# oxfordcontrol/COSMO.jl

Hardware: AMD Instinct MI355X
Metric: ADMM iterations/sec (fp64) at fixed (n,m,nnz,cone) (higher is better)
Workload: dtype f64

## Files before the change

cosmo.jl_amd/_ffi.py:

```python
from __future__ import annotations

import ctypes as C
import os

import numpy as np

_HERE = os.path.dirname(os.path.abspath(__file__))
LIB_PATH = os.path.join(_HERE, "libcosmo_hip.so")
LIB_PATH_F32 = os.path.join(_HERE, "libcosmo_hip_f32.so")

OK = 0
ERR_NAMES = {1: "INVALID", 2: "HIP", 5: "EIG", 6: "UNSUPPORTED", 7: "COMM"}

ZERO, NONNEG, BOX, SOC, PSD_SQUARE, PSD_TRIANGLE = 0, 1, 2, 3, 4, 5
EXP, DUAL_EXP, POW, DUAL_POW = 6, 7, 8, 9
PSD_TRIANGLE_COMPLEX = 10
CUSTOM = 11
KKT_CG, KKT_MINRES_REDUCED, KKT_MINRES, KKT_CG_SR, KKT_CG_JACOBI = 0, 1, 2, 3, 4
KKT_DIRECT = 5
STATUS_NAMES = {0: "Undetermined", 1: "Solved", 2: "Max_iter_reached", 3: "Unsolved", 4: "Primal_infeasible",
                5: "Dual_infeasible", 6: "Time_limit_reached"}
MAT_A, MAT_AT, MAT_P, MAT_OP = 0, 1, 2, 3
MAX_RHO_UPDATES = 64
NUM_KERNEL_CLASSES = 16


from ._abi_structs import ABI_VERSION, AccelParams, Params, ResultStruct

ACCEL_EMPTY, ACCEL_ANDERSON = 0, 1
PSD_PROJECTION_SIGN, PSD_PROJECTION_EIGEN = 0, 1
ACCEL_ANDERSON_TYPE1_RESTARTED, ACCEL_ANDERSON_TYPE1_ROLLING, ACCEL_ANDERSON_TYPE2NE_RESTARTED, ACCEL_ANDERSON_TYPE2NE_ROLLING = 2, 3, 4, 5


class CosmoHipError(RuntimeError):
    def __init__(self, code, msg):
        super().__init__("libcosmo_hip error %d (%s): %s" % (code, ERR_NAMES.get(code, "?"), msg))
        self.code = code


_libs = {}

_PD = C.POINTER(C.c_double)
_PF = C.POINTER(C.c_float)


class _RealPtr:
    """Placeholder in SIGNATURES for `cosmo_hip_real*` (include/cosmo_hip.h): resolved to double* or float* when a library is loaded."""


_PR = _RealPtr
_PI64 = C.POINTER(C.c_int64)
_PI32 = C.POINTER(C.c_int32)

PROJECT_FN = C.CFUNCTYPE(None, C.POINTER(C.c_double), C.c_int64, C.c_void_p)
CONE_TEST_FN = C.CFUNCTYPE(C.c_int32, C.POINTER(C.c_double), C.c_int64, C.c_double, C.c_void_p)
PROJECT_FN_F32 = C.CFUNCTYPE(None, C.POINTER(C.c_float), C.c_int64, C.c_void_p)
CONE_TEST_FN_F32 = C.CFUNCTYPE(C.c_int32, C.POINTER(C.c_float), C.c_int64, C.c_double, C.c_void_p)

SIGNATURES = {
    "cosmo_hip_version": (C.c_int32, []),
    "cosmo_hip_default_params": (None, [C.POINTER(Params)]),
    "cosmo_hip_create": (C.c_int32, [C.POINTER(C.c_void_p), C.c_int32]),
    "cosmo_hip_destroy": (C.c_int32, [C.c_void_p]),
    "cosmo_hip_last_error": (C.c_char_p, [C.c_void_p]),
    "cosmo_hip_set_problem": (C.c_int32, [C.c_void_p, C.c_int64, C.c_int64, _PI64, _PI64, _PR, _PI64, _PI64, _PR, _PR, _PR]),
    "cosmo_hip_set_cones": (C.c_int32, [C.c_void_p, C.c_int64, _PI32, _PI64, _PR, _PR]),
    "cosmo_hip_set_cones_ex": (C.c_int32, [C.c_void_p, C.c_int64, _PI32, _PI64, _PR, _PR, _PR]),
    "cosmo_hip_set_custom_cone": (C.c_int32, [C.c_void_p, C.c_int64, PROJECT_FN, CONE_TEST_FN, CONE_TEST_FN, C.c_void_p]),
    "cosmo_hip_set_params": (C.c_int32, [C.c_void_p, C.POINTER(Params), _PR]),
    "cosmo_hip_update_rho": (C.c_int32, [C.c_void_p, _PR]),
    "cosmo_hip_set_scaling": (C.c_int32, [C.c_void_p, _PR, _PR, C.c_double]),
    "cosmo_hip_set_scaling_full": (C.c_int32, [C.c_void_p, _PR, _PR, _PR, _PR, C.c_double, C.c_double]),
    "cosmo_hip_default_accel_params": (None, [C.POINTER(AccelParams)]),
    "cosmo_hip_set_accelerator": (C.c_int32, [C.c_void_p, C.POINTER(AccelParams)]),
    "cosmo_hip_get_accel_stats": (C.c_int32, [C.c_void_p, _PI64]),
    "cosmo_hip_get_accel_restarts": (C.c_int32, [C.c_void_p, _PI64]),
    "cosmo_hip_scale_ruiz": (C.c_int32, [C.c_void_p, C.c_int64, C.c_double, C.c_double, _PR, _PR, _PD]),
    "cosmo_hip_update_qb": (C.c_int32, [C.c_void_p, _PR, _PR]),
    "cosmo_hip_get_rho_classes": (C.c_int32, [C.c_void_p, _PI32]),
    "cosmo_hip_get_rho_vec": (C.c_int32, [C.c_void_p, _PR]),
    "cosmo_hip_kkt_solve": (C.c_int32, [C.c_void_p, _PR, _PR, _PI64]),
    "cosmo_hip_project": (C.c_int32, [C.c_void_p, _PR, _PI64, _PI32]),
    "cosmo_hip_spmv": (C.c_int32, [C.c_void_p, C.c_int32, _PR, _PR]),
    "cosmo_hip_set_iterates": (C.c_int32, [C.c_void_p, _PR, _PR, _PR]),
    "cosmo_hip_admm_init": (C.c_int32, [C.c_void_p]),
    "cosmo_hip_admm_iterate": (C.c_int32, [C.c_void_p, C.c_int64]),
    "cosmo_hip_admm_iterate_checked": (C.c_int32, [C.c_void_p, C.c_int64, _PI32]),
    "cosmo_hip_residuals": (C.c_int32, [C.c_void_p, _PD]),
    "cosmo_hip_optimize": (C.c_int32, [C.c_void_p, C.POINTER(ResultStruct)]),
    "cosmo_hip_get_iterates": (C.c_int32, [C.c_void_p, _PR, _PR, _PR, _PR]),
    "cosmo_hip_cg_persist_stats": (C.c_int32, [C.c_void_p, _PI64]),
    "cosmo_hip_fold_stats": (C.c_int32, [C.c_void_p, _PI64]),
    "cosmo_hip_kkt_recurrence": (C.c_char_p, [C.c_void_p]),
    "cosmo_hip_ldl_analyze": (C.c_int32, [C.c_int64, C.c_int64, _PI64, _PI64, _PI64, _PI64, _PI64, _PI64]),
    "cosmo_hip_set_kkt_perm": (C.c_int32, [C.c_void_p, C.c_int64, _PI64]),
    "cosmo_hip_direct_info": (C.c_int32, [C.c_void_p, _PI64]),
    "cosmo_hip_polar_dataflow_stats": (C.c_int32, [C.c_void_p, _PD]),
    "cosmo_hip_polar_dataflow_reset_timing": (C.c_int32, [C.c_void_p]),
    "cosmo_hip_get_kkt_solution": (C.c_int32, [C.c_void_p, _PR]),
    "cosmo_hip_get_stats": (C.c_int32, [C.c_void_p, _PI64]),
    "cosmo_hip_set_setup_time": (C.c_int32, [C.c_void_p, C.c_double]),
    "cosmo_hip_get_rho_interval": (C.c_int32, [C.c_void_p, _PI64]),
    "cosmo_hip_time_spmv": (C.c_int32, [C.c_void_p, C.c_int32, C.c_int32, _PD, _PD]),
    "cosmo_hip_set_profiling": (C.c_int32, [C.c_void_p, C.c_int32]),
    "cosmo_hip_get_kernel_times": (C.c_int32, [C.c_void_p, _PD, _PI64]),
    "cosmo_hip_kernel_class_name": (C.c_char_p, [C.c_int32]),
    "cosmo_hip_psd_stats": (C.c_int32, [C.c_void_p, _PI64]),
    "cosmo_hip_set_psd_projection": (C.c_int32, [C.c_void_p, C.c_int32]),
    "cosmo_hip_polar_stats": (C.c_int32, [C.c_void_p, _PI64]),
    "cosmo_hip_polar_streamk_stats": (C.c_int32, [C.c_void_p, _PI64]),
    "cosmo_hip_polar_schedule": (C.c_int32, [C.c_int32, _PD, _PI32]),
    "cosmo_hip_time_psd_product": (C.c_int32, [C.c_void_p, C.c_int32, C.c_int32, _PD, _PD]),
    "cosmo_hip_comm_unique_id": (C.c_int32, [C.POINTER(C.c_uint8)]),
    "cosmo_hip_comm_init": (C.c_int32, [C.c_void_p, C.c_int32, C.c_int32, C.POINTER(C.c_uint8)]),
    "cosmo_hip_comm_destroy": (C.c_int32, [C.c_void_p]),
    "cosmo_hip_set_cone_shard": (C.c_int32, [C.c_void_p, _PI64]),
    "cosmo_hip_polar_depth_stats": (C.c_int32, [C.c_void_p, _PI64]),
    "cosmo_hip_time_krylov": (C.c_int32, [C.c_void_p, C.c_int32, C.POINTER(C.c_double), C.POINTER(C.c_double), C.POINTER(C.c_int32)]),
    "cosmo_hip_comm_selftest": (C.c_int32, [C.c_void_p]),
    "cosmo_hip_comm_allreduce_check": (C.c_int32, [C.c_void_p, C.c_int64, _PI64]),
    "cosmo_hip_comm_init_hostshm": (C.c_int32, [C.c_void_p, C.c_int32, C.c_int32, C.c_char_p]),
    "cosmo_hip_comm_stats": (C.c_int32, [C.c_void_p, _PI64]),
    "cosmo_hip_set_cone_ownership": (C.c_int32, [C.c_void_p, C.c_int64, C.c_int64]),
    "cosmo_hip_set_row_shard": (C.c_int32, [C.c_void_p, _PI64]),
    "cosmo_hip_row_shard_info": (C.c_int32, [C.c_void_p, _PI64]),
    "cosmo_hip_comm_stats_ex": (C.c_int32, [C.c_void_p, _PI64]),
    "cosmo_hip_batch_create": (C.c_int32, [C.POINTER(C.c_void_p), C.c_int32, C.c_int64, C.c_int64, C.c_int64]),
    "cosmo_hip_batch_destroy": (C.c_int32, [C.c_void_p]),
    "cosmo_hip_batch_last_error": (C.c_char_p, [C.c_void_p]),
    "cosmo_hip_batch_set_problem": (C.c_int32, [C.c_void_p, C.c_int64, _PI64, _PI64, _PR, _PI64, _PI64, _PR, _PR, _PR]),
    "cosmo_hip_batch_set_cones": (C.c_int32, [C.c_void_p, C.c_int64, _PI32, _PI64, _PR, _PR]),
    "cosmo_hip_batch_set_cones_ex": (C.c_int32, [C.c_void_p, C.c_int64, _PI32, _PI64, _PR, _PR, _PR]),
    "cosmo_hip_batch_set_scaling": (C.c_int32, [C.c_void_p, C.c_int64, _PR, _PR, C.c_double]),
    "cosmo_hip_batch_set_params": (C.c_int32, [C.c_void_p, C.POINTER(Params)]),
    "cosmo_hip_batch_set_accelerator": (C.c_int32, [C.c_void_p, C.POINTER(AccelParams)]),
    "cosmo_hip_batch_get_accel_stats": (C.c_int32, [C.c_void_p, _PI64]),
    "cosmo_hip_batch_get_rho_classes": (C.c_int32, [C.c_void_p, C.c_int64, _PI32]),
    "cosmo_hip_batch_set_iterates": (C.c_int32, [C.c_void_p, _PR, _PR, _PR]),
    "cosmo_hip_batch_optimize": (C.c_int32, [C.c_void_p, C.POINTER(ResultStruct)]),
    "cosmo_hip_batch_iterate": (C.c_int32, [C.c_void_p, C.c_int64, C.c_int32]),
    "cosmo_hip_batch_get_iterates": (C.c_int32, [C.c_void_p, C.c_int64, _PR, _PR, _PR, _PR]),
    "cosmo_hip_batch_get_counters": (C.c_int32, [C.c_void_p, _PI64]),
    "cosmo_hip_batch_kernel_info": (C.c_int32, [C.c_void_p, _PI64]),
    "cosmo_hip_batch_set_direct": (C.c_int32, [C.c_void_p, C.c_int32, _PI64]),
    "cosmo_hip_batch_direct_info": (C.c_int32, [C.c_void_p, _PI64]),
    "cosmo_hip_batch_direct_counts": (C.c_int32, [C.c_void_p, _PI64]),
    "cosmo_hip_batch_set_scaling_full": (C.c_int32, [C.c_void_p, C.c_int64, _PR, _PR, _PR, _PR, C.c_double, C.c_double]),
    "cosmo_hip_batch_stage_qb": (C.c_int32, [C.c_void_p, C.c_int64, _PR, _PR]),
    "cosmo_hip_batch_apply_updates": (C.c_int32, [C.c_void_p]),
    "cosmo_hip_batch_update_qb": (C.c_int32, [C.c_void_p, C.c_int64, _PI64, _PR, _PR]),
    "cosmo_hip_batch_warm_restart": (C.c_int32, [C.c_void_p]),
    "cosmo_hip_batch_get_qb": (C.c_int32, [C.c_void_p, C.c_int64, _PR, _PR]),
    "cosmo_hip_batch_group_create": (C.c_int32, [C.POINTER(C.c_void_p), C.c_int32, C.c_int64]),
    "cosmo_hip_batch_group_destroy": (C.c_int32, [C.c_void_p]),
    "cosmo_hip_batch_group_last_error": (C.c_char_p, [C.c_void_p]),
    "cosmo_hip_batch_group_set_problem": (C.c_int32, [C.c_void_p, C.c_int64, C.c_int64, C.c_int64, _PI64, _PI64, _PR, _PI64, _PI64, _PR, _PR, _PR]),
    "cosmo_hip_batch_group_set_cones": (C.c_int32, [C.c_void_p, C.c_int64, C.c_int64, _PI32, _PI64, _PR, _PR, _PR]),
    "cosmo_hip_batch_group_set_scaling": (C.c_int32, [C.c_void_p, C.c_int64, _PR, _PR, C.c_double]),
    "cosmo_hip_batch_group_set_scaling_full": (C.c_int32, [C.c_void_p, C.c_int64, _PR, _PR, _PR, _PR, C.c_double, C.c_double]),
    "cosmo_hip_batch_group_set_accelerator": (C.c_int32, [C.c_void_p, C.POINTER(AccelParams)]),
    "cosmo_hip_batch_group_set_direct": (C.c_int32, [C.c_void_p, C.c_int32]),
    "cosmo_hip_batch_group_set_params": (C.c_int32, [C.c_void_p, C.POINTER(Params)]),
    "cosmo_hip_batch_group_class_info": (C.c_int32, [C.c_void_p, _PI64, _PI64, _PI64]),
    "cosmo_hip_batch_group_run_info": (C.c_int32, [C.c_void_p, _PI64]),
    "cosmo_hip_batch_group_get_rho_interval": (C.c_int32, [C.c_void_p, C.c_int64, _PI64]),
# ... 153 lines not shown
            if fn is None:
                return test_t(0)
            return test_t(lambda ptr, dim, tol, _user: 1 if fn(_view(ptr, dim), float(tol)) else 0)

        f32 = self.dtype == np.float32
        proj_t, test_t = (PROJECT_FN_F32, CONE_TEST_FN_F32) if f32 else (PROJECT_FN, CONE_TEST_FN)
        thunks = (proj_t(_proj), _mk(in_dual), _mk(in_pol_recc))
        self._callbacks[int(cone)] = thunks
        self._chk(self.lib.cosmo_hip_set_custom_cone(self._h, int(cone), thunks[0], thunks[1], thunks[2], None))

    def default_params(self):
        return default_params(self.dtype)

    def set_params(self, params, rho_vec=None):
        rv = self._f(rho_vec, self.m, "rho_vec")
        self._chk(self.lib.cosmo_hip_set_params(self._h, C.byref(params), _dp(rv)))

    def update_rho(self, rho_vec):
        rv = self._f(rho_vec, self.m, "rho_vec")
        self._chk(self.lib.cosmo_hip_update_rho(self._h, _dp(rv)))

    def set_accelerator(self, kind=ACCEL_ANDERSON, mem=15, min_mem=3, safeguard=True, safeguard_tol=2.0, start_iter=2, start_accuracy=None):
        ap = AccelParams()
        self.lib.cosmo_hip_default_accel_params(C.byref(ap))
        ap.kind, ap.mem, ap.min_mem, ap.safeguard = int(kind), int(mem), int(min_mem), 1 if safeguard else 0
        ap.safeguard_tol, ap.start_iter = float(safeguard_tol), int(start_iter)
        if start_accuracy is not None:
            ap.start_accuracy = float(start_accuracy)
        self._chk(self.lib.cosmo_hip_set_accelerator(self._h, C.byref(ap)))

    def accel_restarts(self):
        out = np.zeros(2, dtype=np.int64)
        self._chk(self.lib.cosmo_hip_get_accel_restarts(self._h, out.ctypes.data_as(_PI64)))
        return int(out[0]), int(out[1])

    def set_psd_projection(self, mode):
        self._chk(self.lib.cosmo_hip_set_psd_projection(self._h, int(mode)))

    def accel_stats(self):
        out = np.zeros(6, dtype=np.int64)
        self._chk(self.lib.cosmo_hip_get_accel_stats(self._h, out.ctypes.data_as(_PI64)))
        return dict(accelerated=int(out[0]), accepted=int(out[1]), declined=int(out[2]), restarts=int(out[3]), active=bool(out[4]),
                    safeguarding_iter=int(out[5]))

    def scale_ruiz(self, iterations, min_scaling=1e-4, max_scaling=1e4):
        D = np.empty(self.n, dtype=self.dtype); E = np.empty(self.m, dtype=self.dtype); c = C.c_double(1.0)
        self._chk(self.lib.cosmo_hip_scale_ruiz(self._h, int(iterations), float(min_scaling), float(max_scaling), _dp(D), _dp(E), C.byref(c)))
        return D, E, float(c.value)

    def set_scaling(self, Dinv, Einv, cinv):
        self._chk(self.lib.cosmo_hip_set_scaling(self._h, _dp(self._f(Dinv, self.n)), _dp(self._f(Einv, self.m)), float(cinv)))

    def set_scaling_full(self, D, Dinv, E, Einv, c, cinv):
        self._chk(self.lib.cosmo_hip_set_scaling_full(self._h, _dp(self._f(D, self.n)), _dp(self._f(Dinv, self.n)), _dp(self._f(E, self.m)),
                                                      _dp(self._f(Einv, self.m)), float(c), float(cinv)))

    def update_qb(self, q=None, b=None):
        self._chk(self.lib.cosmo_hip_update_qb(self._h, _dp(self._f(q, self.n)), _dp(self._f(b, self.m))))

    def get_rho_classes(self):
        out = np.empty(self.m, dtype=np.int32)
        self._chk(self.lib.cosmo_hip_get_rho_classes(self._h, out.ctypes.data_as(_PI32)))
        return out

    def get_rho_vec(self):
        out = np.empty(self.m, dtype=self.dtype)
        self._chk(self.lib.cosmo_hip_get_rho_vec(self._h, _dp(out)))
        return out

    def kkt_solve(self, rhs):
        rhs = self._f(rhs, self.n + self.m, "rhs")
        lhs = np.empty(self.n + self.m, dtype=self.dtype)
        it = C.c_int64(0)
        self._chk(self.lib.cosmo_hip_kkt_solve(self._h, _dp(lhs), _dp(rhs), C.byref(it)))
        return lhs, it.value

    def project(self, s):
        s = np.array(s, dtype=self.dtype).copy()
        ranks = np.empty(max(self.ncones, 1), dtype=np.int64)
        br = np.empty(max(self.ncones, 1), dtype=np.int32)
        self._chk(self.lib.cosmo_hip_project(self._h, _dp(s), ranks.ctypes.data_as(_PI64), br.ctypes.data_as(_PI32)))
        return s, ranks[:self.ncones], br[:self.ncones]

    def spmv(self, which, x):
        nin = {MAT_A: self.n, MAT_AT: self.m, MAT_P: self.n}[which]
        nout = {MAT_A: self.m, MAT_AT: self.n, MAT_P: self.n}[which]
        x = self._f(x, nin, "x")
        y = np.empty(nout, dtype=self.dtype)
        self._chk(self.lib.cosmo_hip_spmv(self._h, which, _dp(y), _dp(x)))
        return y

    def set_iterates(self, x0=None, s0=None, mu0=None):
        self._chk(self.lib.cosmo_hip_set_iterates(self._h, _dp(self._f(x0, self.n)), _dp(self._f(s0, self.m)), _dp(self._f(mu0, self.m))))

    def admm_init(self):
        self._chk(self.lib.cosmo_hip_admm_init(self._h))

    def admm_iterate(self, n_iters):
        self._chk(self.lib.cosmo_hip_admm_iterate(self._h, int(n_iters)))

    def admm_iterate_checked(self, n_iters):
        st = C.c_int32(0)
        self._chk(self.lib.cosmo_hip_admm_iterate_checked(self._h, int(n_iters), C.byref(st)))
        return st.value

    def set_setup_time(self, seconds):
        self._chk(self.lib.cosmo_hip_set_setup_time(self._h, float(seconds)))

    def rho_interval(self):
        out = np.zeros(2, dtype=np.int64)
        self._chk(self.lib.cosmo_hip_get_rho_interval(self._h, out.ctypes.data_as(_PI64)))
        return int(out[0]), int(out[1])

    def residuals(self):
        out = np.empty(5)
        self._chk(self.lib.cosmo_hip_residuals(self._h, _dp(out)))
        return out

    def optimize(self):
        r = ResultStruct()
        self._chk(self.lib.cosmo_hip_optimize(self._h, C.byref(r)))
        return r

    def get_iterates(self):
        N = self.n + self.m
        w = np.empty(N, dtype=self.dtype); wp = np.empty(N, dtype=self.dtype); s = np.empty(self.m, dtype=self.dtype); mu = np.empty(self.m, dtype=self.dtype)
        self._chk(self.lib.cosmo_hip_get_iterates(self._h, _dp(w), _dp(wp), _dp(s), _dp(mu)))
        return w, wp, s, mu

    def get_kkt_solution(self):
        sol = np.empty(self.n + self.m, dtype=self.dtype)
        self._chk(self.lib.cosmo_hip_get_kkt_solution(self._h, _dp(sol)))
        return sol

    def get_stats(self):
        out = np.zeros(8, dtype=np.int64)
        self._chk(self.lib.cosmo_hip_get_stats(self._h, out.ctypes.data_as(_PI64)))
        keys = ["admm_iters", "kkt_solves", "kkt_iters_total", "kkt_budget_stalls", "spmv_A", "spmv_AT", "spmv_P", "rho_updates"]
        return dict(zip(keys, out.tolist()))

    def cg_persist_stats(self):
        out = np.zeros(8, dtype=np.int64)
        self._chk(self.lib.cosmo_hip_cg_persist_stats(self._h, out.ctypes.data_as(_PI64)))
        return dict(zip(["enabled", "workgroups", "launches", "fallbacks", "tickets", "arrivals", "abort", "lds_per_quarter"], out.tolist()))

    def set_kkt_perm(self, perm):
        if perm is None:
            self._chk(self.lib.cosmo_hip_set_kkt_perm(self._h, 0, None))
            return
        p = np.ascontiguousarray(perm, dtype=np.int64)
        self._chk(self.lib.cosmo_hip_set_kkt_perm(self._h, int(p.size), p.ctypes.data_as(_PI64)))

    def direct_info(self):
        out = np.zeros(8, dtype=np.int64)
        self._chk(self.lib.cosmo_hip_direct_info(self._h, out.ctypes.data_as(_PI64)))
        keys = ["nnz_L", "nnz_stored", "supernodes", "height", "max_width", "factorizations", "positive_pivots", "last_factor_ns"]
        return dict(zip(keys, out.tolist()))

    def kkt_recurrence(self):
        return self.lib.cosmo_hip_kkt_recurrence(self._h).decode()

    def fold_stats(self):
        out = np.zeros(6, dtype=np.int64)
        self._chk(self.lib.cosmo_hip_fold_stats(self._h, out.ctypes.data_as(_PI64)))
        return dict(zip(["enabled", "nnz", "terms", "tiles", "factored_rows", "stored_entries"], out.tolist()))

# ... 389 lines not shown
```

cosmo.jl_amd/csrc/api.hip:

```cpp
#include <stdarg.h>
#include <stdio.h>
#include <string.h>
#include <math.h>
#include <algorithm>
#include <chrono>
#include "internal.h"
#include "device_utils.h"

int32_t cosmo_fail(cosmo_hip_handle* h, int32_t code, const char* fmt, ...) {
  char buf[1024];
  va_list ap;
  va_start(ap, fmt);
  vsnprintf(buf, sizeof buf, fmt, ap);
  va_end(ap);
  if (h) h->err = buf;
  return code;
}

template <class T>
static int32_t dalloc(cosmo_hip_handle* h, T** p, size_t count) {
  if (*p) { (void)hipFree(*p); *p = nullptr; }
  if (count == 0) count = 1;
  HIPCHK(h, hipMalloc((void**)p, count * sizeof(T)));
  HIPCHK(h, hipMemsetAsync(*p, 0, count * sizeof(T), h->stream));
// ... 577 lines not shown
}

extern "C" int32_t cosmo_hip_update_qb(cosmo_hip_handle* h, const real* q, const real* b) {
  ENTER(h);
  if (!h->have_problem) return cosmo_fail(h, COSMO_HIP_ERR_INVALID, "set_problem first");
  if (b && h->row_shard) return cosmo_fail(h, COSMO_HIP_ERR_UNSUPPORTED, "update_qb(b): not available on a row-sharded handle");
  if (q) CHK(h2d(h, h->q, q, (size_t)h->n));
  if (b) {
    CHK(h2d(h, h->b, b, (size_t)h->m));
    if (h->have_cones) {
      std::vector<real> bhost(b, b + h->m);
      CHK(classify_rows(h, bhost));
    }
  }
  return COSMO_HIP_OK;
}

extern "C" int32_t cosmo_hip_get_rho_classes(cosmo_hip_handle* h, int32_t* cls) {
  ENTER(h);
  if (h->row_shard) return cosmo_fail(h, COSMO_HIP_ERR_UNSUPPORTED, "get_rho_classes: not available on a row-sharded handle");
  if (!h->have_cones || !cls) return cosmo_fail(h, COSMO_HIP_ERR_INVALID, "get_rho_classes: not set up");
  return d2h(h, cls, h->rho_cls, (size_t)h->m);
}
extern "C" int32_t cosmo_hip_get_rho_vec(cosmo_hip_handle* h, real* rho_vec) {
  ENTER(h);
  if (h->row_shard) return cosmo_fail(h, COSMO_HIP_ERR_UNSUPPORTED, "get_rho_vec: not available on a row-sharded handle");
  if (!h->have_params || !rho_vec) return cosmo_fail(h, COSMO_HIP_ERR_INVALID, "get_rho_vec: not set up");
  return d2h(h, rho_vec, h->rho, (size_t)h->m);
}

int32_t sync_ctl(cosmo_hip_handle* h) {
  HIPCHK(h, hipMemcpyAsync(h->ctl_host, h->ctl, sizeof(Ctl), hipMemcpyDeviceToHost, h->stream));
  HIPCHK(h, hipStreamSynchronize(h->stream));
  CHK(prof_collect(h));
  if (h->ctl_host->error) return cosmo_fail(h, h->ctl_host->error, "device raised error %d", h->ctl_host->error);
  return COSMO_HIP_OK;
}

extern "C" int32_t cosmo_hip_spmv(cosmo_hip_handle* h, int32_t which, real* y, const real* x) {
  ENTER(h);
  if (h->row_shard) return cosmo_fail(h, COSMO_HIP_ERR_UNSUPPORTED, "spmv: not available on a row-sharded handle");
  if (!h->have_problem || !x || !y) return cosmo_fail(h, COSMO_HIP_ERR_INVALID, "spmv: not set up");
  const CsrDev* M = which == COSMO_HIP_MAT_A ? &h->A : which == COSMO_HIP_MAT_AT ? &h->AT : which == COSMO_HIP_MAT_P ? &h->P : nullptr;
  if (!M) return cosmo_fail(h, COSMO_HIP_ERR_INVALID, "spmv: bad matrix id");
  real* dx = h->io;
  real* dy = h->io + M->ncols;
  if ((long long)M->ncols + M->nrows > 2 * (h->n + h->m)) return cosmo_fail(h, COSMO_HIP_ERR_INVALID, "spmv: staging too small");
  CHK(h2d(h, dx, x, (size_t)M->ncols));
  CHK(launch_spmv_plain(h, *M, dx, dy));
  CHK(d2h(h, y, dy, (size_t)M->nrows));
  h->spmv_calls[which] += 1;
  return COSMO_HIP_OK;
}

extern "C" int32_t cosmo_hip_project(cosmo_hip_handle* h, real* s, int64_t* psd_rank_out, int32_t* soc_branch_out) {
  ENTER(h);
  if (h->row_shard) return cosmo_fail(h, COSMO_HIP_ERR_UNSUPPORTED, "project: not available on a row-sharded handle");
  if (!h->have_cones || (!s && h->m > 0)) return cosmo_fail(h, COSMO_HIP_ERR_INVALID, "project: not set up");
  CHK(h2d(h, h->io, s, (size_t)h->m));
  CHK(launch_project_simple_inplace(h, h->io));
  CHK(launch_soc(h, h->io, 0));
  CHK(cone3_enqueue_project(h, h->io, 0));
  CHK(psd_enqueue_project(h, h->io, false));
  CHK(custom_enqueue_project(h, h->io, 0));
  CHK(comm_enqueue_exchange(h, h->io));
  CHK(d2h(h, s, h->io, (size_t)h->m));
  const size_t nc = h->cones.type.size();
  if (soc_branch_out) {
    for (size_t k = 0; k < nc; ++k) soc_branch_out[k] = -1;
    if (h->nsoc) {
      std::vector<int> br((size_t)h->nsoc);
      CHK(d2h(h, br.data(), h->soc_branch, (size_t)h->nsoc));
      for (int i = 0; i < h->nsoc; ++i) soc_branch_out[h->soc_cone_index[i]] = br[i];
    }
    CHK(cone3_get_branches(h, soc_branch_out));
  }
  if (psd_rank_out) {
    for (size_t k = 0; k < nc; ++k) psd_rank_out[k] = -1;
    CHK(psd_get_ranks(h, psd_rank_out));
    for (size_t k = 0; k < nc; ++k)
      if ((h->cones.type[k] == COSMO_HIP_PSD_SQUARE || h->cones.type[k] == COSMO_HIP_PSD_TRIANGLE) && h->cones.dim[k] == 1)
        psd_rank_out[k] = s[h->cones.off[k]] > R(0.0) ? 1 : 0;
  }
  return COSMO_HIP_OK;
}

static void adapt_budget(cosmo_hip_handle* h) {
  const int kmax = h->ctl_host->cg_k_max;
  int nb = kmax + 2;
  if (nb < 3) nb = 3;
  if (nb > 4096) nb = 4096;
  h->budget = nb;
}

__global__ void k_ctl_reset_kmax(Ctl* ctl) { ctl->cg_k_max = 0; }
__global__ void k_ctl_set_status(Ctl* ctl, int st) { ctl->status = st; ctl->halt = 1; }
static bool inf_due(const cosmo_hip_handle* h, long long it);

static int32_t maybe_infeas_check(cosmo_hip_handle* h, long long it) {
  if (h->ctl_host->status != 0 || !inf_due(h, it)) return COSMO_HIP_OK;
  int32_t st = 0;
  CHK(infeas_check(h, &st));
  if (st != 0) {
    hipLaunchKernelGGL(k_ctl_set_status, dim3(1), dim3(1), 0, h->stream, h->ctl, st);
    CHK(sync_ctl(h));
  }
  return COSMO_HIP_OK;
}

extern "C" int32_t cosmo_hip_kkt_solve(cosmo_hip_handle* h, real* lhs, const real* rhs, int64_t* kkt_iters_out) {
  ENTER(h);
  if (h->row_shard) return cosmo_fail(h, COSMO_HIP_ERR_UNSUPPORTED, "kkt_solve: not available on a row-sharded handle");
  if (!h->have_params || !lhs || !rhs) return cosmo_fail(h, COSMO_HIP_ERR_INVALID, "kkt_solve: not set up");
  CHK(h2d(h, h->ls_x, rhs, (size_t)h->n));
  CHK(h2d(h, h->ls_s, rhs + h->n, (size_t)h->m));
  CHK(kkt_solve_now(h));
  h->host_solves += 1;
  CHK(sync_ctl(h));
  if (kkt_iters_out) *kkt_iters_out = h->ctl_host->cg_k;
  CHK(d2h(h, lhs, h->x_tl, (size_t)h->n));
  CHK(d2h(h, lhs + h->n, h->nu, (size_t)h->m));
  return COSMO_HIP_OK;
}

extern "C" int32_t cosmo_hip_set_iterates(cosmo_hip_handle* h, const real* x0, const real* s0, const real* mu0) {
  ENTER(h);
  if (!h->have_params) return cosmo_fail(h, COSMO_HIP_ERR_INVALID, "set_iterates: set_params first");
  const long long n = h->n, m = h->m;
  const real *dx = nullptr, *ds = nullptr, *dm = nullptr;
  if (h->row_shard) { if (s0) s0 += h->row_lo; if (mu0) mu0 += h->row_lo; }
  if (x0) { CHK(h2d(h, h->ls_x, x0, (size_t)n)); dx = h->ls_x; }
  if (s0) { CHK(h2d(h, h->ls_s, s0, (size_t)m)); ds = h->ls_s; }
  if (mu0) { CHK(h2d(h, h->tmp_m, mu0, (size_t)m)); dm = h->tmp_m; }
  CHK(launch_set_w(h, dx, ds, dm));
  HIPCHK(h, hipMemcpyAsync(h->w_prev, h->w, sizeof(real) * (size_t)(n + m), hipMemcpyDeviceToDevice, h->stream));
  CHK(d2h(h, h->ctl_host, h->ctl, 1));
  Ctl* c = h->ctl_host;
  c->halt = 0; c->status = 0; c->stalled = 0; c->error = 0; c->cg_done = 0; c->cg_k = 0; c->cg_k_max = 0; c->rho_changed = 0;
  c->iter = 0;
  c->r_prim = INFINITY; c->r_dual = INFINITY; c->max_norm_prim = 0; c->max_norm_dual = 0; c->cost = INFINITY;
  CHK(h2d(h, h->ctl, h->ctl_host, 1));
  h->host_iter = 0;
  h->have_iterates = true;
  h->fb_from = h->fb_recorded;
  return COSMO_HIP_OK;
}

static const int FB_LAG = 2;
static void feedback_reset(cosmo_hip_handle* h) { h->fb_from = h->fb_recorded; }
int32_t solve_budget(cosmo_hip_handle* h, int* budget_out) {
  const int R = cosmo_hip_handle::FB_RING;
  bool& used = h->fb_used[(h->host_solves + 1) % R];
  used = false;
  if (h->fb_mode == 1 && !h->fb_k) {
    if (const char* e = getenv("COSMO_HIP_BUDGET_FEEDBACK")) { if (atoi(e) == 0) h->fb_mode = 0; }
    if (h->fb_mode == 1 && hipHostMalloc((void**)&h->fb_k, sizeof(int) * cosmo_hip_handle::FB_RING) != hipSuccess) { (void)hipGetLastError(); h->fb_k = nullptr; h->fb_mode = 0; }
  }
  *budget_out = h->budget;
  if (h->fb_mode != 1 || h->profiling || h->exact_launches) return COSMO_HIP_OK;
  const long long j = h->fb_recorded - FB_LAG;
  const int wide = h->budget + h->budget / 16;
  if (j < h->fb_from || j < 0) { *budget_out = wide > 4096 ? 4096 : wide; return COSMO_HIP_OK; }
  HIPCHK(h, hipEventSynchronize(h->fb_ev[j % R]));
  int kmax = h->fb_k[j % R], kmin = kmax, nv = 1;
  for (long long i = j - 1; i >= h->fb_from && i > j - 4; --i) { const int v = h->fb_k[i % R]; kmax = std::max(kmax, v); kmin = std::min(kmin, v); nv += 1; }
  int b = (nv >= 3) ? kmax + (kmax - kmin) / 2 + kmax / 40 + 3 : kmax + (kmax * 15 + 99) / 100 + 6;
// ... 506 lines not shown
```

cosmo.jl_amd/csrc/internal.h:

```cpp
#pragma once
#include <hip/hip_runtime.h>
#include <stdint.h>
#include <string>
#include <vector>
#include "../../include/cosmo_hip.h"

typedef cosmo_hip_real real;
#ifdef COSMO_HIP_REAL_FLOAT
typedef float2 real2;
#define make_real2 make_float2
#define REAL_EPS 1.1920928955078125e-07f
#define REAL_MAX 3.402823466e+38f
#define REAL_IS_FLOAT 1
#else
typedef double2 real2;
#define make_real2 make_double2
#define REAL_EPS 2.220446049250313e-16
#define REAL_MAX 1.7976931348623157e308
#define REAL_IS_FLOAT 0
#endif
#define R(x) ((real)(x))

#define COSMO_BS 256
#define COSMO_NNZ_PER_BLOCK 2048
// ... 257 lines not shown
int32_t launch_set_w(cosmo_hip_handle* h, const real* x0, const real* s0, const real* mu0);
int32_t launch_recover_mu(cosmo_hip_handle* h);
int32_t launch_rho_from_classes(cosmo_hip_handle* h, real rho0);
int32_t launch_spmv_plain(cosmo_hip_handle* h, const CsrDev& M, const real* x, real* y);
int32_t launch_spmv_A_rho(cosmo_hip_handle* h, int guard, int mode, const real* v, real* out);
int32_t launch_reduced_rhs(cosmo_hip_handle* h, int guard, real* out_rhs);
int32_t launch_cg_upd(cosmo_hip_handle* h, int guard, int k, int n_uc);
int32_t launch_cg_dir_check(cosmo_hip_handle* h, int guard, int kk, int n_rr);
int32_t enqueue_cg_rhs(cosmo_hip_handle* h, int guard);
int32_t enqueue_cg_start(cosmo_hip_handle* h, int guard, real tol_k);
int32_t enqueue_cg_iterations(cosmo_hip_handle* h, int guard, int k_begin, int count);
int32_t enqueue_rhs(cosmo_hip_handle* h, int guard);
int32_t enqueue_y2_only(cosmo_hip_handle* h);
int32_t enqueue_tail(cosmo_hip_handle* h, int loop_mode);
int32_t enqueue_count_solve(cosmo_hip_handle* h);
int32_t enqueue_clear_stall(cosmo_hip_handle* h);
int32_t enqueue_check(cosmo_hip_handle* h, int guard, int mode);
int32_t time_op_apply(cosmo_hip_handle* h, int reps, double* avg_seconds);

int32_t fold_build(cosmo_hip_handle* h, const HostCsr& Am, const std::vector<int>& prp, const std::vector<int>& pcol,
                   const std::vector<real>& pval, int factor_min);
int32_t fold_refresh(cosmo_hip_handle* h);
void fold_free(cosmo_hip_handle* h);
int32_t fold_enqueue_start(cosmo_hip_handle* h, int guard, real tol_k);
int32_t fold_enqueue_iterations(cosmo_hip_handle* h, int guard, int k_begin, int count);

int32_t minres_alloc(cosmo_hip_handle* h);
int32_t minres_enqueue_solve(cosmo_hip_handle* h, int guard, bool from_loop);
int32_t minres_resume(cosmo_hip_handle* h, int extra);
int32_t launch_mr_tail_full(cosmo_hip_handle* h, int loop_mode, const real* xsol);

int32_t ldl_setup(cosmo_hip_handle* h, const std::vector<int64_t>& perm_req);
void ldl_free(cosmo_hip_handle* h);
int32_t ldl_enqueue_refactor(cosmo_hip_handle* h, int cond);
int32_t ldl_refactor_now(cosmo_hip_handle* h, bool inertia);
int32_t ldl_enqueue_solve(cosmo_hip_handle* h, int guard, bool from_loop);
int32_t ldl_info(cosmo_hip_handle* h, int64_t* out);

int32_t sr_alloc(cosmo_hip_handle* h);
void sr_free(cosmo_hip_handle* h);
int32_t sr_enqueue_start(cosmo_hip_handle* h, int guard);
int32_t sr_enqueue_iterations(cosmo_hip_handle* h, int guard, int k_begin, int count);

bool batch_multi_supported(const cosmo_hip_batch* b);
bool batch_multi_needs_ext(const cosmo_hip_batch* b);
int32_t batch_multi_optimize(cosmo_hip_batch** bs, int count, bool ext, cosmo_hip_result* results);

int32_t pcg_setup(cosmo_hip_handle* h, bool* accepted);
void pcg_free(cosmo_hip_handle* h);
int32_t pcg_enqueue_solve(cosmo_hip_handle* h, int guard);

void aa_free(cosmo_hip_handle* h);
bool aa_get_params(const cosmo_hip_handle* h, cosmo_hip_accel_params* out);
bool aa_enabled(const cosmo_hip_handle* h);
bool aa_safeguarded(const cosmo_hip_handle* h);
bool aa_active(const cosmo_hip_handle* h);
int32_t aa_restart(cosmo_hip_handle* h);
void aa_note_rho_restart(cosmo_hip_handle* h);
int32_t aa_begin_solve(cosmo_hip_handle* h);
int32_t aa_enqueue_pre(cosmo_hip_handle* h, long long it, bool* attempted);
int32_t aa_fetch_flags(cosmo_hip_handle* h, int* success, int* declined);
int32_t aa_enqueue_guard(cosmo_hip_handle* h);
int32_t aa_enqueue_reset(cosmo_hip_handle* h);
void aa_count(cosmo_hip_handle* h, int accelerated, int declined);
void aa_check_accuracy_activation(cosmo_hip_handle* h, real r_prim, real r_dual, real max_norm_prim, real max_norm_dual);

int32_t cone3_plan_create(cosmo_hip_handle* h);
void cone3_free(cosmo_hip_handle* h);
int32_t cone3_enqueue_project(cosmo_hip_handle* h, real* s, int guard);
int32_t cone3_enqueue_in_dual_neg(cosmo_hip_handle* h, const real* v, real tol, int* flag);
int32_t cone3_get_branches(cosmo_hip_handle* h, int32_t* out_per_cone);

int32_t custom_plan_create(cosmo_hip_handle* h);
void custom_free(cosmo_hip_handle* h);
int32_t custom_enqueue_project(cosmo_hip_handle* h, real* s, int guard);
int32_t custom_test(cosmo_hip_handle* h, const real* v_dev, int which, real tol, bool* ok);

int32_t polar_plan_create(cosmo_hip_handle* h);
void polar_plan_destroy(cosmo_hip_handle* h);
bool polar_enabled(const cosmo_hip_handle* h);
int32_t polar_enqueue_project(cosmo_hip_handle* h, real* s, int guard);
int32_t polar_enqueue_project_batch(cosmo_hip_handle* h, real* s, int guard);
int32_t polar_adapt(cosmo_hip_handle* h);
bool polar_has_batch(const cosmo_hip_handle* h);
bool polar_has_large(const cosmo_hip_handle* h);

int32_t polar_complex_is_pd(cosmo_hip_handle* h, const real* vec, real sign, real tol, std::vector<int>& ok);

int32_t psd_plan_create(cosmo_hip_handle* h);
void psd_plan_destroy(cosmo_hip_handle* h);
int32_t psd_enqueue_project(cosmo_hip_handle* h, real* s, bool guard);
int32_t psd_get_ranks(cosmo_hip_handle* h, int64_t* rank_per_cone);
int32_t psd_extreme_eigs(cosmo_hip_handle* h, const real* vec, real sign, real tol, std::vector<real>& lam_min);
static inline bool cone_owned(const cosmo_hip_handle* h, long long k) { return h->cone_hi < 0 || (k >= h->cone_lo && k < h->cone_hi); }
int32_t infeas_enqueue_capture(cosmo_hip_handle* h);
int32_t infeas_check(cosmo_hip_handle* h, int32_t* status);
int32_t comm_enqueue_exchange(cosmo_hip_handle* h, real* s);
int32_t comm_allgather_rows(cosmo_hip_handle* h, real* full);
int32_t comm_allreduce_sum(cosmo_hip_handle* h, real* buf, size_t count);
int32_t comm_allreduce_host(cosmo_hip_handle* h, double* vals, int count, int op );
int comm_nranks(const cosmo_hip_handle* h);
int comm_rank(const cosmo_hip_handle* h);
int32_t comm_allreduce_flag(cosmo_hip_handle* h, int* flag);
int32_t comm_set_partition(cosmo_hip_handle* h, const int64_t* first_cone, const char* who);
void comm_my_range(const cosmo_hip_handle* h, long long* cone_lo, long long* cone_hi, long long* row_lo, long long* row_hi);
int32_t rs_enqueue_cg_rhs(cosmo_hip_handle* h, int guard);
int32_t rs_get_iterates(cosmo_hip_handle* h, real* w, real* w_prev, real* s, real* mu);
void rs_free(cosmo_hip_handle* h);
extern "C" int32_t cosmo_hip_comm_destroy(cosmo_hip_handle* h);
```

cosmo.jl_amd/csrc/psd.hip:

```cpp
#include "device_utils.h"
#include <algorithm>
#include <math.h>
#include <stdlib.h>

#include "psd_internal.h"
#include "psd16.h"
#include "psdwg.h"

__global__ __launch_bounds__(COSMO_BS) void k_psd_tiny(const Ctl* __restrict__ ctl, int guard, int ncones,
                                                       const int* __restrict__ list, const PsdConeDev* __restrict__ cones,
                                                       real* __restrict__ s, int* __restrict__ rank, int* __restrict__ flags,
                                                       int mode, real sign, real* __restrict__ eigmin) {
  if (guard && ctl->halt) return;
  __shared__ __attribute__((aligned(16))) unsigned char wsb[COSMO_BS / 64][(PSD16_WS_BYTES + 15) / 16 * 16];
  const int lane = threadIdx.x & 63, wv = threadIdx.x >> 6;
  const int widx = blockIdx.x * (COSMO_BS / 64) + wv;
  if (widx >= ncones) return;
  const PsdConeDev cn = cones[list[widx]];
  const Psd16Ws ws = psd16_ws_at(wsb[wv]);
  int nonconv = 0;
  real lm = 0.0;
  const int rk = psd16_wave(s + cn.off, cn.d, cn.kind, ws, lane, mode, sign, &lm, &nonconv);
  if (nonconv && lane == 0) atomicOr(&flags[1], 1);
  if (mode == 1) { if (lane == 0) eigmin[list[widx]] = lm; return; }
// ... 313 lines not shown
      p->d_pj_groups.push_back(dptr);
    }
  }
  HIPCHK(h, hipMalloc((void**)&p->G, std::max<long long>(1, p->gsize) * sizeof(real)));
  HIPCHK(h, hipMalloc((void**)&p->colw, std::max(1, p->ncolw) * sizeof(real)));
  HIPCHK(h, hipMalloc((void**)&p->cshift, p->cones.size() * sizeof(real)));
  HIPCHK(h, hipMalloc((void**)&p->rank, p->cones.size() * sizeof(int)));
  HIPCHK(h, hipMalloc((void**)&p->flags, 4 * sizeof(int)));
  HIPCHK(h, hipMalloc((void**)&p->eigmin, p->cones.size() * sizeof(real)));
  HIPCHK(h, hipMemset(p->rank, 0, p->cones.size() * sizeof(int)));
  HIPCHK(h, hipMemset(p->flags, 0, 4 * sizeof(int)));
  return polar_plan_create(h);
}

static int32_t psd_large_sweeps(cosmo_hip_handle* h, int n, int nbmax) {
  PsdPlan* p = h->psd;
  int sweep = 0;
  for (; sweep < PSD_MAX_SWEEPS; ++sweep) {
    HIPCHK(h, hipMemsetAsync(p->flags, 0, sizeof(int), h->stream));
    for (int st = -1; st < nbmax - 1; ++st)
      hipLaunchKernelGGL(k_psd_step, dim3(nbmax / 2, n), dim3(PSD_STEP_WAVES * 64), 0, h->stream, p->d_large, p->d_cones, p->G,
                         p->cshift, st, p->flags, p->tol_factor);
    int fl = 0;
    HIPCHK(h, hipMemcpyAsync(&fl, p->flags, sizeof(int), hipMemcpyDeviceToHost, h->stream));
    HIPCHK(h, hipStreamSynchronize(h->stream));
    if (!fl) break;
  }
  p->last_large_sweeps = sweep + 1;
  if (sweep >= PSD_MAX_SWEEPS) return cosmo_fail(h, COSMO_HIP_ERR_EIG, "Jacobi eigensolver did not converge in %d sweeps", PSD_MAX_SWEEPS);
  return COSMO_HIP_OK;
}

bool psd_needs_sync(const cosmo_hip_handle* h) { return h->psd && !h->psd->large.empty() && !polar_has_large(h); }

int32_t psd_enqueue_project(cosmo_hip_handle* h, real* s, bool guard_b) {
  PsdPlan* p = h->psd;
  if (!p || p->cones.empty()) return COSMO_HIP_OK;
  const int guard = guard_b ? 1 : 0;
  prof_begin(h, KC_PSD);
  HIPCHK(h, hipMemsetAsync(p->rank, 0, p->cones.size() * sizeof(int), h->stream));
  if (!p->tiny.empty()) {
    const int n = (int)p->tiny.size();
    hipLaunchKernelGGL(k_psd_tiny, dim3((n + COSMO_BS / 64 - 1) / (COSMO_BS / 64)), dim3(COSMO_BS), 0, h->stream, h->ctl, guard, n,
                       p->d_tiny, p->d_cones, s, p->rank, p->flags, 0, 1.0, p->eigmin);
  }
  for (size_t gi = 0; gi < p->pj_groups.size(); ++gi) {
    const int n = (int)p->pj_groups[gi].size();
    const int* lst = p->d_pj_groups[gi];
    hipLaunchKernelGGL(k_psd_populate, dim3(8, n), dim3(COSMO_BS), 0, h->stream, h->ctl, guard, lst, p->d_cones, s, p->G, p->cshift, 1.0, 0);
    switch (p->pj_waves[gi]) {
      case 16: hipLaunchKernelGGL((k_psd_jacobi_wg<16>), dim3(n), dim3(1024), 0, h->stream, h->ctl, guard, lst, p->d_cones, p->G, p->cshift, p->flags, p->tol_factor, p->dbg); break;
      default: hipLaunchKernelGGL((k_psd_jacobi_wg<4>), dim3(n), dim3(256), 0, h->stream, h->ctl, guard, lst, p->d_cones, p->G, p->cshift, p->flags, p->tol_factor, p->dbg); break;
    }
    hipLaunchKernelGGL(k_psd_colscale, dim3(4, n), dim3(COSMO_BS), 0, h->stream, h->ctl, guard, lst, p->d_cones, p->G, p->cshift, p->colw, p->rank);
    int maxtiles = 1;
    for (int idx : p->pj_groups[gi]) { const int nt = p->cones[idx].ld / 16; maxtiles = std::max(maxtiles, nt * (nt + 1) / 2); }
    hipLaunchKernelGGL(k_psd_syrk, dim3((maxtiles + 3) / 4, n), dim3(COSMO_BS), 0, h->stream, h->ctl, guard, lst, p->d_cones, p->G, s);
  }
  if (polar_has_batch(h)) CHK(polar_enqueue_project_batch(h, s, guard));
  if (polar_has_large(h)) CHK(polar_enqueue_project(h, s, guard));
  if (!p->large.empty() && !(polar_has_large(h) && p->large_by_polar)) {
    if (guard) {
      CHK(sync_ctl(h));
      if (h->ctl_host->halt) { prof_end(h); return COSMO_HIP_OK; }
    }
    const int n = (int)p->large.size();
    int nbmax = 0;
    for (int idx : p->large) nbmax = std::max(nbmax, p->cones[idx].nb);
    hipLaunchKernelGGL(k_psd_populate, dim3(64, n), dim3(COSMO_BS), 0, h->stream, h->ctl, 0, p->d_large, p->d_cones, s, p->G, p->cshift, 1.0, 0);
    CHK(psd_large_sweeps(h, n, nbmax));
    hipLaunchKernelGGL(k_psd_colscale, dim3(128, n), dim3(COSMO_BS), 0, h->stream, h->ctl, 0, p->d_large, p->d_cones, p->G, p->cshift, p->colw, p->rank);
    int maxtiles = 1;
    for (int idx : p->large) { const int nt = p->cones[idx].ld / 16; maxtiles = std::max(maxtiles, nt * (nt + 1) / 2); }
    hipLaunchKernelGGL(k_psd_syrk, dim3(std::min(8192, (maxtiles + 3) / 4), n), dim3(COSMO_BS), 0, h->stream, h->ctl, 0, p->d_large, p->d_cones, p->G, s);
  }
  prof_end(h);
  HIPCHK(h, hipGetLastError());
  return COSMO_HIP_OK;
}

int32_t psd_get_ranks(cosmo_hip_handle* h, int64_t* rank_per_cone) {
  PsdPlan* p = h->psd;
  if (!p || p->cones.empty()) return COSMO_HIP_OK;
  std::vector<int> r(p->cones.size());
  int fl[4] = {0, 0, 0, 0};
  HIPCHK(h, hipMemcpyAsync(r.data(), p->rank, r.size() * sizeof(int), hipMemcpyDeviceToHost, h->stream));
  HIPCHK(h, hipMemcpyAsync(fl, p->flags, sizeof fl, hipMemcpyDeviceToHost, h->stream));
  HIPCHK(h, hipStreamSynchronize(h->stream));
  if (fl[1]) return cosmo_fail(h, COSMO_HIP_ERR_EIG, "Jacobi eigensolver did not converge");
  for (size_t i = 0; i < p->cones.size(); ++i) rank_per_cone[p->cones[i].cone_index] = r[i];
  return COSMO_HIP_OK;
}

extern "C" int32_t cosmo_hip_psd_stats(cosmo_hip_handle* h, int64_t out[4]) {
  if (!h || !out) return COSMO_HIP_ERR_INVALID;
  out[0] = out[1] = out[2] = out[3] = 0;
  PsdPlan* p = h->psd;
  if (!p || p->cones.empty()) return COSMO_HIP_OK;
  int fl[4] = {0, 0, 0, 0};
  HIPCHK(h, hipMemcpyAsync(fl, p->flags, sizeof fl, hipMemcpyDeviceToHost, h->stream));
  HIPCHK(h, hipStreamSynchronize(h->stream));
  out[0] = fl[2]; out[1] = p->last_large_sweeps; out[2] = fl[1]; out[3] = (int64_t)p->cones.size();
  return COSMO_HIP_OK;
}


int32_t psd_extreme_eigs(cosmo_hip_handle* h, const real* vec, real sign, real tol, std::vector<real>& lam_min) {
  PsdPlan* p = h->psd;
  lam_min.clear();
  if (!p || p->cones.empty()) return COSMO_HIP_OK;
  real* v = const_cast<real*>(vec);
  if (!p->tiny.empty()) {
    const int n = (int)p->tiny.size();
    hipLaunchKernelGGL(k_psd_tiny, dim3((n + COSMO_BS / 64 - 1) / (COSMO_BS / 64)), dim3(COSMO_BS), 0, h->stream, h->ctl, 0, n, p->d_tiny,
                       p->d_cones, v, p->rank, p->flags, 1, sign, p->eigmin);
  }
  for (size_t gi = 0; gi < p->wg_groups.size(); ++gi) {
    const int n = (int)p->wg_groups[gi].size();
    const int* lst = p->d_wg_groups[gi];
    hipLaunchKernelGGL(k_psd_populate, dim3(8, n), dim3(COSMO_BS), 0, h->stream, h->ctl, 0, lst, p->d_cones, vec, p->G, p->cshift, sign, 1);
    if (p->wg_waves[gi] == 16)
      hipLaunchKernelGGL((k_psd_jacobi_wg<16>), dim3(n), dim3(1024), 0, h->stream, h->ctl, 0, lst, p->d_cones, p->G, p->cshift, p->flags, p->tol_factor, 0);
    else
      hipLaunchKernelGGL((k_psd_jacobi_wg<4>), dim3(n), dim3(256), 0, h->stream, h->ctl, 0, lst, p->d_cones, p->G, p->cshift, p->flags, p->tol_factor, 0);
    hipLaunchKernelGGL(k_psd_eigmin, dim3(n), dim3(COSMO_BS), 0, h->stream, lst, p->d_cones, p->G, p->cshift, p->eigmin);
  }
  if (!p->large.empty()) {
    const int n = (int)p->large.size();
    int nbmax = 0;
    for (int idx : p->large) nbmax = std::max(nbmax, p->cones[idx].nb);
    hipLaunchKernelGGL(k_psd_populate, dim3(64, n), dim3(COSMO_BS), 0, h->stream, h->ctl, 0, p->d_large, p->d_cones, vec, p->G, p->cshift, sign, 1);
    CHK(psd_large_sweeps(h, n, nbmax));
    hipLaunchKernelGGL(k_psd_eigmin, dim3(n), dim3(COSMO_BS), 0, h->stream, p->d_large, p->d_cones, p->G, p->cshift, p->eigmin);
  }
  HIPCHK(h, hipGetLastError());
  lam_min.resize(p->cones.size());
  HIPCHK(h, hipMemcpyAsync(lam_min.data(), p->eigmin, sizeof(real) * lam_min.size(), hipMemcpyDeviceToHost, h->stream));
  HIPCHK(h, hipStreamSynchronize(h->stream));
  if (!p->cplx.empty()) {
    std::vector<int> ok;
    CHK(polar_complex_is_pd(h, vec, sign, tol, ok));
    for (size_t q = 0; q < p->cplx.size(); ++q) lam_min[p->cplx[q]] = ok[q] ? 0.0 : -INFINITY;
  }
  return COSMO_HIP_OK;
}
```

cosmo.jl_amd/csrc/psd_polar.hip:

```cpp
#include "psd_internal.h"
#include <math.h>
#include <stdlib.h>
#include <string.h>
#include <algorithm>
#include <mutex>

#define PK 16
#ifndef POLAR_PREFETCH_DEPTH
#define POLAR_PREFETCH_DEPTH 2
#endif
#define PLD 80

struct PolarCone {
  int idx;
  int off, d, kind;
  int ts;
  int sk;
  int skg, skc;
  int ld;
  long long woff;
};

struct BatchCone { long long woff; int off, d, kind, ld, idx, ts; };

struct SkSync { unsigned ticket; unsigned timeout; unsigned pad[14]; unsigned flag[1]; };
struct PolarDev {
  int gate;
  int rounds;
  int verified;
  int unverified;
  int projections;
  int pad[3];
  real err_last, err_max;
};

static const real kPolarLift[3] = {3.8438259784376458, -2.5414431444903771, 0.42553478492344637};
#define POLAR_NFIN 5
static const real kPolarFinish[POLAR_NFIN][3] = {
    {3.4931704678738202, -2.370790022242379, 0.42240833954524776},
    {2.7077959763108326, -2.015093165601975, 0.45683257965863566},
    {1.9693651031668091, -1.3512768962961363, 0.3852630352029357},
    {1.875, -1.25, 0.375},
    {1.875, -1.25, 0.375}};
#define POLAR_RLIFT 3
#define POLAR_NFIN_LARGE (REAL_IS_FLOAT ? 4 : POLAR_NFIN)
#define POLAR_RLIFT_LARGE (REAL_IS_FLOAT ? 4 : POLAR_RLIFT)

struct PolarPlan {
  std::vector<PolarCone> cones;
  real* W = nullptr;
  real* parts = nullptr;
  real* nrm = nullptr;
  int k_lift = REAL_IS_FLOAT ? 5 : 9;
  int max_rounds = 2;
  int rescale = 1;
  int batch_occ = 3;
  real tol_factor = 8.0;
  PolarDev* dev = nullptr;
  PolarDev seen;
  long long launches[4] = {0, 0, 0, 0};
  int streamk = 0;
  real* sk_scratch = nullptr;
  SkSync* sk_sync = nullptr;
  int sk_gmax = 0;
  unsigned sk_base = 0, sk_epoch = 0;
  int products_last_large = 0, products_last_batch = 0;
  std::vector<BatchCone> bcones;
  BatchCone* d_bcones = nullptr;
  int4* d_btiles = nullptr;
  int nbtiles = 0, nbtiles96 = 0;
  int speculate = 0;
  int* gate_host = nullptr;
  int batch_wave = 0;
  int batch_ragged = 1;
  void* d_rtiles = nullptr;
  int nrtiles = 0;
  int dataflow = 0;
  void* d_df_tiles = nullptr;
  int* d_df_cone_nt = nullptr;
  unsigned* d_df_sync = nullptr;
  int df_xoff[9] = {0, 0, 0, 0, 0, 0, 0, 0, 0};
  int df_grid = 0;
  long long df_launches = 0, df_timed = 0;
  int df_nprod = 0;
  double df_seconds = 0.0;
  hipEvent_t df_ev[2] = {nullptr, nullptr};
  int df_ev_pending = 0;
  void* h_rtiles = nullptr;
  void* rep_host = nullptr;
  void* d_rtiles_rep = nullptr;
  int nrep = 0;
  long long repair_launch_tiles = 0, repair_trains = 0;
  double batch_flops_performed = 0.0, batch_flops_useful = 0.0;
  int batch_ts96 = 0;
  real* BW = nullptr;
  real* bparts = nullptr;
  real* bnrm = nullptr;
  int* bgate = nullptr;
  int adapt = 0;
  int compact_repair = 1;
  std::vector<int> bk, bstreak, bm;
  int* d_lgate = nullptr;
  int* d_ubuf = nullptr;
  int* bgate_host = nullptr;
  int lgate_kmax = -1;
  long long depth_fail = 0, depth_down = 0, depth_proj = 0;
  int seen_proj_batch = 0;
  std::vector<int> lk, lstreak, lm;
  int seen_proj_large = 0;
  double wprod_last = 0.0;
};
#define POLAR_LIFT_CAP 18

extern "C" int32_t cosmo_hip_polar_schedule(int32_t k_lift, double* abc, int32_t* nsteps) {
  if (k_lift < 0 || k_lift > 64 || !nsteps) return COSMO_HIP_ERR_INVALID;
  *nsteps = k_lift + POLAR_NFIN;
  if (!abc) return COSMO_HIP_OK;
  for (int t = 0; t < k_lift; ++t) for (int q = 0; q < 3; ++q) abc[3 * t + q] = (double)kPolarLift[q];
  for (int t = 0; t < POLAR_NFIN; ++t) for (int q = 0; q < 3; ++q) abc[3 * (k_lift + t) + q] = (double)kPolarFinish[t][q];
  return COSMO_HIP_OK;
}

namespace {

__device__ __forceinline__ long long svec_index(int i, int j) { return (long long)j * (j + 1) / 2 + i; }


__device__ __forceinline__ real polar_read(const real* __restrict__ x, int kind, int d, int i, int j) {
  const real isq2 = 0.70710678118654752440;
  if (kind == COSMO_HIP_PSD_TRIANGLE) {
    const int a = i < j ? i : j, b = i < j ? j : i;
    const real t = x[svec_index(a, b)];
    return (a == b) ? t : isq2 * t;
  }
  if (kind == COSMO_HIP_PSD_SQUARE) {
    const int a = i < j ? i : j, b = i < j ? j : i;
    return (x[(long long)b * d + a] + x[(long long)a * d + b]) / R(2.0);
  }
  const int r = d / 2;
  const int bi = i >= r, bj = j >= r, ii = i - bi * r, jj = j - bj * r;
  const int a = ii < jj ? ii : jj, b = ii < jj ? jj : ii;
  if (bi == bj) { const real t = x[svec_index(a, b)]; return (a == b) ? t : isq2 * t; }
  if (ii == jj) return 0.0;
  real im = isq2 * x[(long long)r * (r + 1) / 2 + (long long)b * (b - 1) / 2 + a];
  if (ii > jj) im = -im;
  return (bi == 1) ? im : -im;
}
__device__ __forceinline__ void polar_write(real* __restrict__ x, int kind, int d, int i, int j, real v) {
  const real sq2 = 1.41421356237309504880;
  if (kind == COSMO_HIP_PSD_TRIANGLE) { x[svec_index(i, j)] = (i == j) ? v : sq2 * v; return; }
  if (kind == COSMO_HIP_PSD_SQUARE) { x[(long long)j * d + i] = v; x[(long long)i * d + j] = v; return; }
  const int r = d / 2;
  if (j < r) { x[svec_index(i, j)] = (i == j) ? v : sq2 * v; return; }
  if (i < r) { const int jj = j - r; if (i < jj) x[(long long)r * (r + 1) / 2 + (long long)jj * (jj - 1) / 2 + i] = sq2 * (-v); }
}

__global__ __launch_bounds__(COSMO_BS) void k_polar_populate(const Ctl* __restrict__ ctl, int guard, PolarCone cn, const real* __restrict__ s,
                                                             real* __restrict__ X, real* __restrict__ parts) {
  if (guard && ctl->halt) return;
  __shared__ real red[COSMO_BS / 64];
  const real* x = s + cn.off;
  const int d = cn.d, ld = cn.ld;
  real acc = 0.0;
  for (int j = blockIdx.x; j < ld; j += gridDim.x) {
    for (int i = threadIdx.x; i < ld; i += COSMO_BS) {
      real v = 0.0;
      if (i < d && j < d) { v = polar_read(x, cn.kind, d, i, j); acc += v * v; }
      X[(long long)j * ld + i] = v;
    }
  }
  acc = block_sum(acc, red);
  if (threadIdx.x == 0) parts[blockIdx.x] = acc;
}

__global__ __launch_bounds__(COSMO_BS) void k_polar_scale(const Ctl* __restrict__ ctl, int guard, long long n, int nparts, const real* __restrict__ parts,
                                                          const real* __restrict__ X, real* __restrict__ U, real* __restrict__ nrm_out) {
  if (guard && ctl->halt) return;
  __shared__ real red[COSMO_BS / 64];
  const real nf = sqrt(reduce_partials_sum(parts, nparts, red));
  const real inv = (nf > R(0.0)) ? R(2.0) / nf : R(0.0);
  if (blockIdx.x == 0 && threadIdx.x == 0) *nrm_out = nf;
// ... 514 lines not shown
  const int i0 = td.i0, j0 = td.j0;
  __amdgpu_buffer_rsrc_t rs = __builtin_amdgcn_make_buffer_rsrc((void*)base, 0, SC1 ? (int)(4 * n2 * (long long)sizeof(real)) : 0, 0x00020000);
  const int offA = (int)(ia * n2) + td.i0, offB = (int)(ib * n2) + td.j0;
#ifndef POLAR_LAB_NO_MAINLOOP
  switch (nsl) {
    case 4: symm_mainloop_r<4, (OCC >= 4 ? 1 : 2), SC1>(A, B, ld, i0, j0, nk, smem, acc, oa, ob, pre_last, rs, offA, offB RT_ARG); break;
    case 3: symm_mainloop_r<3, (OCC >= 4 ? 1 : 2), SC1>(A, B, ld, i0, j0, nk, smem, acc, oa, ob, pre_last, rs, offA, offB RT_ARG); break;
    case 2: symm_mainloop_r<2, (OCC >= 4 ? 1 : 2), SC1>(A, B, ld, i0, j0, nk, smem, acc, oa, ob, pre_last, rs, offA, offB RT_ARG); break;
    case 1: symm_mainloop_r<1, (OCC >= 4 ? 1 : 2), SC1>(A, B, ld, i0, j0, nk, smem, acc, oa, ob, pre_last, rs, offA, offB RT_ARG); break;
    default: symm_mainloop_r<0, (OCC >= 4 ? 1 : 2), SC1>(A, B, ld, i0, j0, nk, smem, acc, oa, ob, pre_last, rs, offA, offB RT_ARG); break;
  }
#else
  (void)A; (void)B; (void)nk; (void)pre_last;
#endif
#ifdef POLAR_LAB_NO_EPILOGUE
  if (lane == 0) C[(long long)j0 * ld + i0 + wv] = acc[0][0] + acc[1][0] + acc[2][0] + acc[3][0];
  return;
#endif
  const unsigned long long t_main = RT_NOW();
  (void)t_main; (void)t_start;
  (void)xi; (void)xj;
  {
    const int lj = lane & 15;
#pragma unroll
    for (int sl = 0; sl < 4; ++sl) {
      if (sl < nsl) {
        const int j = ob[sl] + lj;
        const bool dblk = diag && (oa[sl] == ob[sl]);
        real v[4];
        if (EPI == 1) {
          real c[4];
#pragma unroll
          for (int q = 0; q < 4; ++q) {
            const int i = oa[sl] + ACC_ROW(lane, q);
            const bool ok = !(dblk && i > j);
            const real* cp = Cin + (ok ? (long long)(i0 + i) * ld + j0 + j : 0);
            c[q] = SC1 ? __hip_atomic_load(cp, __ATOMIC_RELAXED, __HIP_MEMORY_SCOPE_AGENT) : *cp;
            if (!ok) c[q] = R(0.0);
          }
#pragma unroll
          for (int q = 0; q < 4; ++q) v[q] = alpha * acc[sl][q] + beta * c[q];
        } else {
#pragma unroll
          for (int q = 0; q < 4; ++q) v[q] = acc[sl][q];
        }
#pragma unroll
        for (int q = 0; q < 4; ++q) {
          const int i = oa[sl] + ACC_ROW(lane, q);
          if (!(dblk && i > j)) C[(long long)(j0 + j) * ld + i0 + i] = v[q];
        }
#pragma unroll
        for (int q = 0; q < 4; ++q) {
          const int i = oa[sl] + ACC_ROW(lane, q);
          if (!(dblk && i >= j)) C[(long long)(i0 + i) * ld + j0 + j] = v[q];
        }
      }
    }
  }
#ifdef POLAR_LAB_TIMING
  { const unsigned long long t_end = RT_NOW();
    RT_ADD(0, t_start); RT_ADD(1, t_first); RT_ADD(2, t_main); RT_ADD(3, t_end); RT_ADD(4, nk);
    if (threadIdx.x == 0 && blockIdx.x < RT_MAXT) g_rtw[blockIdx.x] = wall_clock64() - w_start; }
#endif
}

template <int EPI, int OCC>
__global__ __launch_bounds__(256) __attribute__((amdgpu_waves_per_eu(OCC, OCC))) void k_symm_gemm_batch_r(const Ctl* __restrict__ ctl, int guard, const int* __restrict__ gate,
                                                         const RTile* __restrict__ tiles, const BatchCone* __restrict__ cones, real* __restrict__ W,
                                                         int ia, int ib, int icin, int ic, real alpha, real beta) {
  extern __shared__ real smem[];
  const RTile td = tiles[blockIdx.x];
  const int halted = guard ? ctl->halt : 0;
  if (halted) return;
  if (td.cone < 0) return;
  if (gate && !gate[td.cone]) return;
  (void)cones;
  ragged_tile<EPI, OCC>(td, W, ia, ib, icin, ic, alpha, beta, smem, []() {});
}

struct DfProd { int ia, ib, icin, ic, epi, pad; real alpha, beta; };
#define DF_MAX_PROD 64
struct DfArgs { DfProd prod[DF_MAX_PROD]; int nprod; int xoff[9]; };
#define DF_SYNC_DONE 144
__device__ __forceinline__ unsigned df_xcc_id() { unsigned x; asm volatile("s_getreg_b32 %0, hwreg(HW_REG_XCC_ID)" : "=s"(x)); return x & 7u; }
__device__ __forceinline__ unsigned df_ld(const unsigned* p) { return __hip_atomic_load(p, __ATOMIC_RELAXED, __HIP_MEMORY_SCOPE_AGENT); }
#define DF_RMW(ptr) __hip_atomic_fetch_add((ptr), 1u, __ATOMIC_RELAXED, __HIP_MEMORY_SCOPE_AGENT)
template <int OCC>
__global__ __launch_bounds__(256) __attribute__((amdgpu_waves_per_eu(OCC, OCC))) void k_polar_dataflow(Ctl* __restrict__ ctl, int guard, const RTile* __restrict__ tiles,
                                                         const int* __restrict__ cone_nt, unsigned* __restrict__ sync, real* __restrict__ W, const DfArgs a) {
  extern __shared__ real smem[];
  __shared__ unsigned s_item;
  __shared__ int s_fail;
  if (guard && ctl->halt) return;
  const int x = (int)df_xcc_id();
  const int x0 = a.xoff[x];
  const unsigned n_x = (unsigned)(a.xoff[x + 1] - x0);
  const unsigned total = n_x * (unsigned)a.nprod;
  const bool wave0 = __builtin_amdgcn_readfirstlane(threadIdx.x >> 6) == 0;
  if (wave0) { if (threadIdx.x == 0) { s_fail = 0; s_item = (n_x > 0) ? DF_RMW(sync + 16 * x) : 0u; } }
  int prev_cone = -1;
  unsigned nxt = 0;
  bool first = true;
  for (;;) {
    if (wave0) {
      if (threadIdx.x == 0) {
        if (prev_cone >= 0) (void)DF_RMW(sync + DF_SYNC_DONE + prev_cone);
        if (!first) s_item = nxt;
      }
    }
    first = false;
    __syncthreads();
    const unsigned item = __builtin_amdgcn_readfirstlane(s_item);
    if (item >= total) break;
    const unsigned p = item / n_x, t = item - p * n_x;
    const RTile td = tiles[x0 + t];
    if (p > 0) {
      if (wave0) {
        if (threadIdx.x == 0) {
          const unsigned target = p * (unsigned)cone_nt[td.cone];
          const unsigned* cnt = sync + DF_SYNC_DONE + td.cone;
          long sp = 0;
          while (df_ld(cnt) < target) {
            __builtin_amdgcn_s_sleep(1);
            ++sp;
            if ((sp & 255) == 0 && df_ld(sync + 128)) { s_fail = 1; break; }
            if (sp > (1L << 20)) { s_fail = 1; __hip_atomic_store(sync + 128, 1u, __ATOMIC_RELAXED, __HIP_MEMORY_SCOPE_AGENT); ctl->error = COSMO_HIP_ERR_HIP; break; }
          }
        }
      }
      __syncthreads();
      if (__builtin_amdgcn_readfirstlane(s_fail)) break;
    }
    const DfProd pr = a.prod[p];
    auto hook = [&]() { if (wave0) { if (threadIdx.x == 0) nxt = DF_RMW(sync + 16 * x); } };
    if (pr.epi) ragged_tile<1, OCC, true>(td, W, pr.ia, pr.ib, pr.icin, pr.ic, pr.alpha, pr.beta, smem, hook);
    else ragged_tile<0, OCC, true>(td, W, pr.ia, pr.ib, pr.icin, pr.ic, pr.alpha, pr.beta, smem, hook);
    asm volatile("s_waitcnt vmcnt(0)" ::: "memory");
    __syncthreads();
    prev_cone = td.cone;
  }
}
#ifdef POLAR_LAB_TIMING
}
extern "C" void cosmo_dbg_ragged_timing(unsigned long long* out ) {
  (void)hipDeviceSynchronize();
  (void)hipMemcpyFromSymbol(out, HIP_SYMBOL(g_rt), sizeof(unsigned long long) * RT_MAXT * 5);
}
extern "C" void cosmo_dbg_ragged_wall(unsigned long long* out ) {
  (void)hipDeviceSynchronize();
  (void)hipMemcpyFromSymbol(out, HIP_SYMBOL(g_rtw), sizeof(unsigned long long) * RT_MAXT);
}
namespace {
#endif

#define WT_DEPTH 4
#define WT_SPITCH 66
template <int EPI>
__global__ __launch_bounds__(64) __attribute__((amdgpu_waves_per_eu(2, 2))) void k_symm_gemm_batch_w(const Ctl* __restrict__ ctl, int guard, const int* __restrict__ gate,
                                                         const int4* __restrict__ tiles, const BatchCone* __restrict__ cones, real* __restrict__ W,
                                                         int ia, int ib, int icin, int ic, real alpha, real beta) {
  if (guard && ctl->halt) return;
  const int4 td = tiles[blockIdx.x];
  if (td.x < 0) return;
  if (gate && !gate[td.x]) return;
  __shared__ real strip[16 * WT_SPITCH];
  const BatchCone bc = cones[td.x];
  const int ld = bc.ld;
  const long long n2 = (long long)ld * ld;
  real* base = W + bc.woff;
  const real* __restrict__ A = base + ia * n2;
  const real* __restrict__ B = base + ib * n2;
  const real* __restrict__ Cin = base + icin * n2;
  real* __restrict__ C = base + ic * n2;
  const int ti = td.y, tj = td.z, i0 = ti * 64, j0 = tj * 64;
  const int kext = ((bc.d + 31) / 32) * 32;
  const bool diag = (ti == tj);
  const int lane = threadIdx.x, l15 = lane & 15, lk = lane >> 4;
  v4d acc[4][4];
#pragma unroll
  for (int a = 0; a < 4; ++a)
#pragma unroll
    for (int b = 0; b < 4; ++b) acc[a][b] = v4d{0.0, 0.0, 0.0, 0.0};
  const real* pa = A + (long long)lk * ld + i0 + l15;
  const real* pb = B + (long long)lk * ld + j0 + l15;
  const long long kstep = 4LL * ld;
  const int nsteps = kext / 4;
  real fi[WT_DEPTH][4], fj[WT_DEPTH][4];
#define WT_LOAD(SLOT, S)                                                                  \
  {                                                                                       \
    const long long o_ = (long long)(S) * kstep;                                          \
    _Pragma("unroll") for (int t_ = 0; t_ < 4; ++t_) { fi[SLOT][t_] = pa[o_ + 16 * t_]; fj[SLOT][t_] = pb[o_ + 16 * t_]; } \
  }
#define WT_MMA(SLOT, DG)                                                                  \
  {                                                                                       \
    _Pragma("unroll") for (int a_ = 0; a_ < 4; ++a_)                                      \
      _Pragma("unroll") for (int b_ = 0; b_ < 4; ++b_)                                    \
        if (!(DG) || b_ <= a_) acc[a_][b_] = MFMA_REAL(fj[SLOT][a_], fi[SLOT][b_], acc[a_][b_]); \
  }
#define WT_LOOP(DG)                                                                       \
  {                                                                                       \
    int s0 = 0;                                                                           \
    for (; s0 + 4 < nsteps; s0 += 4) {                                                    \
      WT_LOAD(3, s0 + 3) WT_MMA(0, DG)                                                    \
      WT_LOAD(0, s0 + 4) WT_MMA(1, DG)                                                    \
      WT_LOAD(1, s0 + 5) WT_MMA(2, DG)                                                    \
      WT_LOAD(2, s0 + 6) WT_MMA(3, DG)                                                    \
    }                                                                                     \
    WT_LOAD(3, s0 + 3) WT_MMA(0, DG) WT_MMA(1, DG) WT_MMA(2, DG) WT_MMA(3, DG)            \
  }
  WT_LOAD(0, 0) WT_LOAD(1, 1) WT_LOAD(2, 2)
  if (diag) WT_LOOP(1) else WT_LOOP(0)
#undef WT_LOOP
#undef WT_LOAD
#undef WT_MMA
#pragma unroll
  for (int a = 0; a < 4; ++a) {
    real cin[4][4];
    if (EPI == 1) {
#pragma unroll
      for (int b = 0; b < 4; ++b)
#pragma unroll
        for (int q = 0; q < 4; ++q) {
// ... 53 lines not shown
  q->sk_base += (unsigned)G;
  q->launches[2] += 1;
}
static void symm_gemm(cosmo_hip_handle* h, int guard, const int* gate, int ts, int sk, int epi, const real* A, const real* B, const real* Cin, real* C,
                      int ld, real alpha, real beta, int skg = 0, int skc = 8) {
  if (sk == 3) {
    if (epi) launch_symm_gemm_sk<1>(h, guard, gate, A, B, Cin, C, ld, alpha, beta, skg, skc); else launch_symm_gemm_sk<0>(h, guard, gate, A, B, Cin, C, ld, alpha, beta, skg, skc);
    return;
  }
  if (ts == 96 && sk == 2) { if (epi) launch_symm_gemm<1, 96, 2>(h, guard, gate, A, B, Cin, C, ld, alpha, beta); else launch_symm_gemm<0, 96, 2>(h, guard, gate, A, B, Cin, C, ld, alpha, beta); }
  else if (ts == 96) { if (epi) launch_symm_gemm<1, 96, 1>(h, guard, gate, A, B, Cin, C, ld, alpha, beta); else launch_symm_gemm<0, 96, 1>(h, guard, gate, A, B, Cin, C, ld, alpha, beta); }
  else { if (epi) launch_symm_gemm<1, 64, 1>(h, guard, gate, A, B, Cin, C, ld, alpha, beta); else launch_symm_gemm<0, 64, 1>(h, guard, gate, A, B, Cin, C, ld, alpha, beta); }
}

__global__ __launch_bounds__(COSMO_BS) void k_polar_sumsq(const Ctl* __restrict__ ctl, int guard, const int* __restrict__ gate, long long n,
                                                          const real* __restrict__ G, real* __restrict__ parts) {
  if (guard && ctl->halt) return;
  if (gate && !*gate) return;
  __shared__ real red[COSMO_BS / 64];
  real acc = 0.0;
  for (long long i = (long long)blockIdx.x * COSMO_BS + threadIdx.x; i < n; i += (long long)gridDim.x * COSMO_BS) { const real v = G[i]; acc += v * v; }
  acc = block_sum(acc, red);
  if (threadIdx.x == 0) parts[blockIdx.x] = acc;
}
__global__ __launch_bounds__(COSMO_BS) void k_polar_rescale(const Ctl* __restrict__ ctl, int guard, long long n, int nparts, const real* __restrict__ parts,
                                                            real* __restrict__ U, real* __restrict__ Y) {
  if (guard && ctl->halt) return;
  __shared__ real red[COSMO_BS / 64];
  const real yf = sqrt(reduce_partials_sum(parts, nparts, red));
  real g = (yf > R(0.0)) ? R(2.0) / sqrt(yf) : R(1.0);
  if (!(g >= R(1.0)) || !(g <= REAL_MAX)) g = R(1.0);
  const real g2 = g * g;
  for (long long i = (long long)blockIdx.x * COSMO_BS + threadIdx.x; i < n; i += (long long)gridDim.x * COSMO_BS) { U[i] = U[i] * g; Y[i] = Y[i] * g2; }
}
__global__ __launch_bounds__(COSMO_BS) void k_polar_decide(const Ctl* __restrict__ ctl, int guard, PolarDev* __restrict__ pd, int round, int last, int nparts,
                                                           const real* __restrict__ parts, const real* __restrict__ nrm, real tol) {
  if (guard && ctl->halt) return;
  if (round > 0 && !pd->gate) return;
  __shared__ real red[COSMO_BS / 64];
  const real g2 = reduce_partials_sum(parts, nparts, red);
  if (threadIdx.x != 0) return;
  const real nf = *nrm;
  const real err = (nf > R(0.0)) ? R(0.5) * sqrt(g2) / nf : R(0.0);
  const bool ok = !(err > tol);
  pd->err_last = err;
  if (err > pd->err_max || err != err) pd->err_max = err;
  if (round == 0) pd->projections += 1; else pd->rounds += 1;
  if (ok) { pd->verified += 1; pd->gate = 0; }
  else if (last) { pd->unverified += 1; pd->gate = 0; }
  else pd->gate = 1;
}

__global__ __launch_bounds__(COSMO_BS) void k_polar_finish(const Ctl* __restrict__ ctl, int guard, PolarCone cn, const real* __restrict__ X,
                                                           const real* __restrict__ H, const real* __restrict__ U, real* __restrict__ s,
                                                           real* __restrict__ tparts) {
  if (guard && ctl->halt) return;
  __shared__ real red[COSMO_BS / 64];
  real* x = s + cn.off;
  const int d = cn.d, ld = cn.ld;
  real tr = 0.0;
  for (int j = blockIdx.x; j < d; j += gridDim.x) {
    for (int i = threadIdx.x; i <= j; i += COSMO_BS) {
      const long long o = (long long)j * ld + i;
      const real v = (X[o] + H[o]) / R(2.0);
      polar_write(x, cn.kind, d, i, j, v);
      const real u = U[o];
      tr += (i == j) ? (u + u * u) : R(2.0) * u * u;
    }
  }
  tr = block_sum(tr, red);
  if (threadIdx.x == 0) tparts[blockIdx.x] = tr;
}
__global__ __launch_bounds__(COSMO_BS) void k_polar_rank(const Ctl* __restrict__ ctl, int guard, int d, int nparts, const real* __restrict__ tparts,
                                                         int* __restrict__ rank_out, int kind) {
  if (guard && ctl->halt) return;
  __shared__ real red[COSMO_BS / 64];
  const real tr = reduce_partials_sum(tparts, nparts, red);
  (void)d;
  if (threadIdx.x == 0) *rank_out = (int)llround(tr / (kind == COSMO_HIP_PSD_TRIANGLE_COMPLEX ? R(4.0) : R(2.0)));
}

#define BPX 16
__global__ __launch_bounds__(COSMO_BS) void k_bpolar_populate(const Ctl* __restrict__ ctl, int guard, const BatchCone* __restrict__ cones,
                                                              const real* __restrict__ s, real* __restrict__ W, real* __restrict__ parts) {
  if (guard && ctl->halt) return;
  __shared__ real red[COSMO_BS / 64];
  const BatchCone cn = cones[blockIdx.y];
  const real* x = s + cn.off;
  real* X = W + cn.woff;
  const int d = cn.d, ld = cn.ld;
  real acc = 0.0;
  for (int j = blockIdx.x; j < ld; j += gridDim.x) {
    for (int i = threadIdx.x; i < ld; i += COSMO_BS) {
      real v = 0.0;
      if (i < d && j < d) { v = polar_read(x, cn.kind, d, i, j); acc += v * v; }
      X[(long long)j * ld + i] = v;
    }
  }
  acc = block_sum(acc, red);
  if (threadIdx.x == 0) parts[(size_t)blockIdx.y * 2 * BPX + blockIdx.x] = acc;
}
__global__ __launch_bounds__(COSMO_BS) void k_bpolar_scale(const Ctl* __restrict__ ctl, int guard, const BatchCone* __restrict__ cones,
                                                           const real* __restrict__ parts, real* __restrict__ W, real* __restrict__ bnrm,
                                                           const int* __restrict__ ubuf) {
  if (guard && ctl->halt) return;
  const BatchCone cn = cones[blockIdx.y];
  real nf2 = 0.0;
  for (int k = 0; k < BPX; ++k) nf2 += parts[(size_t)blockIdx.y * 2 * BPX + k];
  const real nf = sqrt(nf2);
  const real inv = (nf > R(0.0)) ? R(2.0) / nf : R(0.0);
  if (blockIdx.x == 0 && threadIdx.x == 0) bnrm[blockIdx.y] = nf;
  const long long n2 = (long long)cn.ld * cn.ld;
  const real* X = W + cn.woff;
  real* U = W + cn.woff + (ubuf ? ubuf[blockIdx.y] : 1) * n2;
  for (long long i = (long long)blockIdx.x * COSMO_BS + threadIdx.x; i < n2; i += (long long)gridDim.x * COSMO_BS) U[i] = X[i] * inv;
}
__global__ __launch_bounds__(COSMO_BS) void k_bpolar_finish(const Ctl* __restrict__ ctl, int guard, const BatchCone* __restrict__ cones,
                                                            real* __restrict__ W, int iu, real* __restrict__ s, real* __restrict__ parts) {
  if (guard && ctl->halt) return;
  __shared__ real red[COSMO_BS / 64];
  const BatchCone cn = cones[blockIdx.y];
  const long long n2 = (long long)cn.ld * cn.ld;
  const real* X = W + cn.woff;
  const real* U = W + cn.woff + iu * n2;
  const real* H = W + cn.woff + 3 * n2;
  real* x = s + cn.off;
  const int d = cn.d, ld = cn.ld;
  real tr = 0.0;
  for (int j = blockIdx.x; j < d; j += gridDim.x) {
    for (int i = threadIdx.x; i <= j; i += COSMO_BS) {
      const long long o = (long long)j * ld + i;
      const real v = (X[o] + H[o]) / R(2.0);
      polar_write(x, cn.kind, d, i, j, v);
      const real u = U[o];
      tr += (i == j) ? (u + u * u) : R(2.0) * u * u;
    }
  }
  tr = block_sum(tr, red);
  if (threadIdx.x == 0) parts[(size_t)blockIdx.y * 2 * BPX + BPX + blockIdx.x] = tr;
}
__global__ void k_bpolar_rank(const Ctl* __restrict__ ctl, int guard, int n, const BatchCone* __restrict__ cones, const real* __restrict__ parts,
                              int* __restrict__ rank) {
  if (guard && ctl->halt) return;
  const int c = blockIdx.x * blockDim.x + threadIdx.x;
  if (c >= n) return;
  real tr = 0.0;
  for (int k = 0; k < BPX; ++k) tr += parts[(size_t)c * 2 * BPX + BPX + k];
  rank[cones[c].idx] = (int)llround(tr / (cones[c].kind == COSMO_HIP_PSD_TRIANGLE_COMPLEX ? R(4.0) : R(2.0)));
}

__global__ __launch_bounds__(COSMO_BS) void k_bpolar_sumsq(const Ctl* __restrict__ ctl, int guard, const int* __restrict__ gate, const BatchCone* __restrict__ cones,
                                                           const real* __restrict__ W, int ig, real* __restrict__ vparts) {
  if (guard && ctl->halt) return;
  if (gate && !gate[blockIdx.y]) return;
  __shared__ real red[COSMO_BS / 64];
  const BatchCone cn = cones[blockIdx.y];
  const long long n2 = (long long)cn.ld * cn.ld;
  const real* G = W + cn.woff + ig * n2;
  real acc = 0.0;
  for (long long i = (long long)blockIdx.x * COSMO_BS + threadIdx.x; i < n2; i += (long long)gridDim.x * COSMO_BS) { const real v = G[i]; acc += v * v; }
  acc = block_sum(acc, red);
  if (threadIdx.x == 0) vparts[(size_t)blockIdx.y * BPX + blockIdx.x] = acc;
}
__global__ __launch_bounds__(COSMO_BS) void k_bpolar_decide(const Ctl* __restrict__ ctl, int guard, PolarDev* __restrict__ pd, int* __restrict__ bgate, int round,
                                                            int last, int n, const BatchCone* __restrict__ cones, const real* __restrict__ vparts,
                                                            const real* __restrict__ bnrm, real tol_factor) {
  if (guard && ctl->halt) return;
  if (round > 0 && !pd->gate) return;
  __shared__ real red[COSMO_BS / 64];
  real emax = 0.0, nfail = 0.0, nchk = 0.0;
  for (int c = threadIdx.x; c < n; c += COSMO_BS) {
    if (round > 0 && !bgate[c]) continue;
    real g2 = 0.0;
    for (int k = 0; k < BPX; ++k) g2 += vparts[(size_t)c * BPX + k];
    const real nf = bnrm[c];
    const real err = (nf > R(0.0)) ? R(0.5) * sqrt(g2) / nf : R(0.0);
    const bool ok = !(err > tol_factor * cones[c].d * PSD_EPS);
    bgate[c] = (!ok && !last) ? 1 : 0;
    nchk += 1.0;
    if (!ok) nfail += 1.0;
    emax = (err > emax || err != err) ? err : emax;
  }
  emax = block_max(emax, red);
  nfail = block_sum(nfail, red);
  nchk = block_sum(nchk, red);
  if (threadIdx.x != 0) return;
  pd->err_last = emax;
  if (emax > pd->err_max || emax != emax) pd->err_max = emax;
  if (round == 0) pd->projections += 1; else pd->rounds += 1;
  if (nfail == R(0.0)) { pd->verified += 1; pd->gate = 0; }
  else if (last) { pd->unverified += 1; pd->gate = 0; }
  else pd->gate = 1;
  (void)nchk;
}

}

void polar_plan_destroy(cosmo_hip_handle* h) {
  PolarPlan* q = static_cast<PolarPlan*>(h->psd_polar);
  if (!q) return;
  if (q->W) (void)hipFree(q->W);
  if (q->parts) (void)hipFree(q->parts);
  if (q->nrm) (void)hipFree(q->nrm);
  if (q->gate_host) (void)hipHostFree(q->gate_host);
  if (q->sk_scratch) (void)hipFree(q->sk_scratch);
  if (q->sk_sync) (void)hipFree(q->sk_sync);
  if (q->d_bcones) (void)hipFree(q->d_bcones);
  if (q->d_btiles) (void)hipFree(q->d_btiles);
  if (q->d_rtiles) (void)hipFree(q->d_rtiles);
  if (q->d_rtiles_rep) (void)hipFree(q->d_rtiles_rep);
  if (q->rep_host) (void)hipHostFree(q->rep_host);
  free(q->h_rtiles);
  if (q->BW) (void)hipFree(q->BW);
  if (q->bparts) (void)hipFree(q->bparts);
  if (q->bnrm) (void)hipFree(q->bnrm);
  if (q->bgate) (void)hipFree(q->bgate);
  if (q->d_lgate) (void)hipFree(q->d_lgate);
  if (q->d_ubuf) (void)hipFree(q->d_ubuf);
  if (q->bgate_host) (void)hipHostFree(q->bgate_host);
  if (q->d_df_tiles) (void)hipFree(q->d_df_tiles);
  if (q->d_df_cone_nt) (void)hipFree(q->d_df_cone_nt);
  if (q->d_df_sync) (void)hipFree(q->d_df_sync);
  if (q->df_ev[0]) { (void)hipEventDestroy(q->df_ev[0]); (void)hipEventDestroy(q->df_ev[1]); }
  if (q->dev) (void)hipFree(q->dev);
  delete q;
  h->psd_polar = nullptr;
}

bool polar_enabled(const cosmo_hip_handle* h) { return h->psd_polar != nullptr; }

int32_t polar_plan_create(cosmo_hip_handle* h) {
  polar_plan_destroy(h);
  PsdPlan* p = h->psd;
  if (!p) return COSMO_HIP_OK;
  std::vector<int> large_list, batch_list = p->polar_batch;
  bool jac = h->psd_mode == 1;
  if (const char* e = getenv("COSMO_HIP_PSD_LARGE")) jac = (e[0] == 'j');
  if (!jac) large_list = p->large;
  p->large_by_polar = !jac;
  for (int idx : p->cplx) { if (p->cones[idx].d > 256) large_list.push_back(idx); else batch_list.push_back(idx); }
  const bool use_large = !large_list.empty(), use_batch = !batch_list.empty();
  if (!use_large && !use_batch) return COSMO_HIP_OK;
  PolarPlan* q = new PolarPlan();
  h->psd_polar = q;
  if (const char* e = getenv("COSMO_HIP_POLAR_KLIFT")) q->k_lift = std::min(40, std::max(0, atoi(e)));
  if (const char* e = getenv("COSMO_HIP_POLAR_ADAPT")) q->adapt = atoi(e) ? 1 : 0;
  if (const char* e = getenv("COSMO_HIP_POLAR_COMPACT_REPAIR")) q->compact_repair = atoi(e) ? 1 : 0;
  if (const char* e = getenv("COSMO_HIP_POLAR_RESCALE")) q->rescale = atoi(e) ? 1 : 0;
  if (const char* e = getenv("COSMO_HIP_POLAR_STREAMK")) q->streamk = atoi(e) ? 1 : 0;
  if (const char* e = getenv("COSMO_HIP_POLAR_BATCH_TS96")) q->batch_ts96 = atoi(e) ? 1 : 0;
  if (const char* e = getenv("COSMO_HIP_POLAR_BATCH_WAVE")) q->batch_wave = atoi(e) ? 1 : 0;
  q->speculate = (large_list.size() > 2) ? 1 : 0;
  if (const char* e = getenv("COSMO_HIP_POLAR_SPECULATE")) q->speculate = atoi(e) ? 1 : 0;
  HIPCHK(h, hipHostMalloc((void**)&q->gate_host, 8 * sizeof(int), hipHostMallocDefault));
  for (int i = 0; i < 8; ++i) q->gate_host[i] = 0;
  if (const char* e = getenv("COSMO_HIP_POLAR_ROUNDS")) q->max_rounds = std::min(8, std::max(0, atoi(e)));
  HIPCHK(h, hipMalloc((void**)&q->dev, sizeof(PolarDev)));
  HIPCHK(h, hipMemset(q->dev, 0, sizeof(PolarDev)));
  memset(&q->seen, 0, sizeof(PolarDev));
  if (use_large) {
    long long woff = 0;
    for (int idx : large_list) {
      const PsdConeDev& c = p->cones[idx];
      PolarCone pc;
      pc.idx = idx; pc.off = c.off; pc.d = c.d; pc.kind = c.kind;
      long long best = -1; pc.ts = 64;
      for (int ts : {64, 96}) {
        const long long nt = (c.d + ts - 1) / ts, tiles = nt * (nt + 1) / 2;
        const long long cost = ((tiles + 255) / 256) * (long long)ts * ts;
        if (best < 0 || cost < best) { best = cost; pc.ts = ts; }
      }
      if (const char* e = getenv("COSMO_HIP_POLAR_TS")) { const int v = atoi(e); if (v == 64 || v == 96) pc.ts = v; }
      pc.ld = ((c.d + pc.ts - 1) / pc.ts) * pc.ts;
      { const long long nt = pc.ld / pc.ts; pc.sk = (pc.ts == 96 && nt * (nt + 1) / 2 <= 256) ? 2 : 1; }
      if (const char* e = getenv("COSMO_HIP_POLAR_SK")) { const int v = atoi(e); if (v == 1 || (v == 2 && pc.ts == 96)) pc.sk = v; }
      pc.skg = 0; pc.skc = 8;
      if (q->streamk) {
        pc.ts = SKG_TS; pc.sk = 3;
        pc.ld = ((c.d + pc.ts - 1) / pc.ts) * pc.ts;
        const long long nt = pc.ld / pc.ts, tiles = nt * (nt + 1) / 2, nk = pc.ld / PK;
        pc.skc = tiles >= 64 ? 8 : 1;
        const long long units_min = (tiles / pc.skc) * nk;
        long long per = std::min<long long>(512 / pc.skc, std::max<long long>(1, units_min / 4));
        if (const char* e = getenv("COSMO_HIP_POLAR_SKG")) { const long long v = atoll(e) / pc.skc; if (v >= 1 && v <= 1024 / pc.skc) per = std::min(v, std::max<long long>(1, units_min)); }
        pc.skg = (int)(per * pc.skc);
        q->sk_gmax = std::max(q->sk_gmax, pc.skg);
      }
      pc.woff = woff;
      woff += 4LL * pc.ld * pc.ld;
      q->cones.push_back(pc);
    }
    HIPCHK(h, hipMalloc((void**)&q->W, sizeof(real) * (size_t)woff));
    HIPCHK(h, hipMalloc((void**)&q->parts, sizeof(real) * 2 * COSMO_MAX_PARTIALS * q->cones.size()));
    HIPCHK(h, hipMalloc((void**)&q->nrm, sizeof(real) * q->cones.size()));
    if (q->sk_gmax > 0) {
      const size_t slot = (size_t)SKG_TS * SKG_TS;
      HIPCHK(h, hipMalloc((void**)&q->sk_scratch, sizeof(real) * slot * (size_t)q->sk_gmax));
      const size_t sb = sizeof(SkSync) + sizeof(unsigned) * (size_t)q->sk_gmax;
      HIPCHK(h, hipMalloc((void**)&q->sk_sync, sb));
      HIPCHK(h, hipMemset(q->sk_sync, 0, sb));
    }
  }
  if (use_batch) {
    long long woff = 0;
    std::vector<int4> tiles;
    for (int idx : batch_list) {
      const PsdConeDev& c = p->cones[idx];
      BatchCone bc;
      bc.off = c.off; bc.d = c.d; bc.kind = c.kind; bc.idx = idx;
      bc.ts = (q->batch_ts96 && ((c.d > 64 && c.d <= 96) || (c.d > 128 && c.d <= 192))) ? 96 : 64;
      bc.ld = ((c.d + bc.ts - 1) / bc.ts) * bc.ts;
      bc.woff = woff;
      woff += 4LL * bc.ld * bc.ld;
      q->bcones.push_back(bc);
    }
    std::vector<int> order(q->bcones.size());
    for (size_t i = 0; i < order.size(); ++i) order[i] = (int)i;
    std::stable_sort(order.begin(), order.end(), [&](int a, int b) { return q->bcones[a].ld > q->bcones[b].ld; });
    int count[2] = {0, 0};
    for (int cls = 0; cls < 2; ++cls) {
      const int ts = cls == 0 ? 64 : 96;
      std::vector<int4> tl;
      if (getenv("COSMO_HIP_POLAR_BATCH_FLAT")) {
        for (int ci : order) {
          if (q->bcones[ci].ts != ts) continue;
          const int nt = q->bcones[ci].ld / ts;
          for (int tj = 0; tj < nt; ++tj) for (int ti = 0; ti <= tj; ++ti) tl.push_back(int4{ci, ti, tj, 0});
        }
      } else {
        std::vector<std::vector<int4>> xl(8);
        long long load[8] = {0, 0, 0, 0, 0, 0, 0, 0};
        for (int ci : order) {
          if (q->bcones[ci].ts != ts) continue;
          const int nt = q->bcones[ci].ld / ts;
          int x = 0;
          for (int t = 1; t < 8; ++t) if (load[t] < load[x]) x = t;
          for (int tj = 0; tj < nt; ++tj) for (int ti = 0; ti <= tj; ++ti) xl[x].push_back(int4{ci, ti, tj, 0});
          load[x] += (long long)nt * (nt + 1) / 2 * q->bcones[ci].ld;
        }
        size_t maxlen = 0;
        for (int x = 0; x < 8; ++x) maxlen = std::max(maxlen, xl[x].size());
        tl.assign(8 * maxlen, int4{-1, 0, 0, 0});
        for (int x = 0; x < 8; ++x) for (size_t sl = 0; sl < xl[x].size(); ++sl) tl[8 * sl + x] = xl[x][sl];
      }
      count[cls] = (int)tl.size();
      tiles.insert(tiles.end(), tl.begin(), tl.end());
    }
    q->nbtiles = count[0]; q->nbtiles96 = count[1];
    if (const char* e = getenv("COSMO_HIP_POLAR_BATCH_RAGGED")) q->batch_ragged = atoi(e) ? 1 : 0;
    if (q->batch_ts96 || q->batch_wave) q->batch_ragged = 0;
    q->batch_flops_performed = q->batch_flops_useful = 0.0;
    for (const BatchCone& bc : q->bcones) q->batch_flops_useful += (double)bc.d * bc.d * (bc.d + 1.0);
    if (q->batch_ragged) {
      std::vector<std::vector<RTile>> xl(8);
      long long load[8] = {0, 0, 0, 0, 0, 0, 0, 0};
      for (int ci : order) {
        const BatchCone& bc = q->bcones[ci];
        const int nb16 = (bc.d + 15) / 16, nt = (nb16 + 3) / 4;
        std::vector<int> start(nt + 1, 0);
        for (int t = 0; t < nt; ++t) start[t + 1] = start[t] + nb16 / nt + (t < nb16 % nt ? 1 : 0);
        int x = 0;
        for (int t = 1; t < 8; ++t) if (load[t] < load[x]) x = t;
        for (int tj = 0; tj < nt; ++tj)
          for (int ti = 0; ti <= tj; ++ti) {
            const int ei = start[ti + 1] - start[ti], ej = start[tj + 1] - start[tj], dg = (ti == tj) ? 1 : 0;
            RTile rt; rt.cone = ci; rt.i0 = 16 * start[ti]; rt.j0 = 16 * start[tj]; rt.ext = ei | (ej << 8) | (dg << 16);
            rt.ld = bc.ld; rt.d = bc.d; rt.woff = bc.woff;
            if (rt.i0 + 64 > bc.ld || rt.j0 + 64 > bc.ld) return cosmo_fail(h, COSMO_HIP_ERR_INVALID, "ragged tile exceeds the leading dimension");
            xl[x].push_back(rt);
            const int nblk = dg ? ei * (ei + 1) / 2 : ei * ej, slots = (nblk + 3) / 4;
            load[x] += (long long)slots * nb16;
            q->batch_flops_performed += 2.0 * 256.0 * nblk * 16.0 * nb16;
          }
      }
      int sort_tiles = 1;
      if (const char* e = getenv("COSMO_HIP_POLAR_BATCH_SORT")) sort_tiles = atoi(e) ? 1 : 0;
      if (sort_tiles) {
        auto cost = [](const RTile& t) {
          const int ei = t.ext & 255, ej = (t.ext >> 8) & 255, dg = (t.ext >> 16) & 1;
          const int nblk = dg ? ei * (ei + 1) / 2 : ei * ej, slots = (nblk + 3) / 4;
          return (long long)((t.d + 15) / 16) * (10 * slots + 2) + 125;
        };
        for (int x = 0; x < 8; ++x) std::stable_sort(xl[x].begin(), xl[x].end(), [&](const RTile& a, const RTile& b) { return cost(a) > cost(b); });
      }
      size_t maxlen = 0;
      for (int x = 0; x < 8; ++x) maxlen = std::max(maxlen, xl[x].size());
      std::vector<RTile> rl(8 * std::max<size_t>(maxlen, 1), RTile{-1, 0, 0, 0, 0, 0, 0});
      for (int x = 0; x < 8; ++x) for (size_t sl = 0; sl < xl[x].size(); ++sl) rl[8 * sl + x] = xl[x][sl];
      q->nrtiles = (int)rl.size();
      {
        std::vector<RTile> dl;
        std::vector<int> cnt(q->bcones.size(), 0);
        for (int x = 0; x < 8; ++x) { q->df_xoff[x] = (int)dl.size(); for (const RTile& t : xl[x]) { dl.push_back(t); cnt[(size_t)t.cone] += 1; } }
        q->df_xoff[8] = (int)dl.size();
        if (dl.empty()) dl.push_back(RTile{-1, 0, 0, 0, 0, 0, 0});
        HIPCHK(h, hipMalloc((void**)&q->d_df_tiles, sizeof(RTile) * dl.size()));
        HIPCHK(h, hipMemcpy(q->d_df_tiles, dl.data(), sizeof(RTile) * dl.size(), hipMemcpyHostToDevice));
        HIPCHK(h, hipMalloc((void**)&q->d_df_cone_nt, sizeof(int) * std::max<size_t>(cnt.size(), 1)));
        HIPCHK(h, hipMemcpy(q->d_df_cone_nt, cnt.data(), sizeof(int) * cnt.size(), hipMemcpyHostToDevice));
        HIPCHK(h, hipMalloc((void**)&q->d_df_sync, sizeof(unsigned) * (DF_SYNC_DONE + cnt.size())));
        hipDeviceProp_t prop;
        HIPCHK(h, hipGetDeviceProperties(&prop, h->device));
        q->df_grid = std::max(1, prop.multiProcessorCount) * 4;
        { int nmin = INT32_MAX; for (int x = 0; x < 8; ++x) nmin = std::min(nmin, q->df_xoff[x + 1] - q->df_xoff[x]); q->dataflow = (nmin >= q->df_grid / 8) ? 1 : 0; }
        if (const char* e = getenv("COSMO_HIP_POLAR_DATAFLOW")) q->dataflow = atoi(e) ? 1 : 0;
        if (const char* e = getenv("COSMO_HIP_POLAR_DATAFLOW_GRID")) { const int v = atoi(e); if (v >= 8 && v <= 8192) q->df_grid = v; }
        (void)hipFuncSetAttribute((const void*)k_polar_dataflow<4>, hipFuncAttributeMaxDynamicSharedMemorySize, GemmCfg<64>::SMEM); }
      HIPCHK(h, hipMalloc((void**)&q->d_rtiles, sizeof(RTile) * rl.size()));
      HIPCHK(h, hipMemcpy(q->d_rtiles, rl.data(), sizeof(RTile) * rl.size(), hipMemcpyHostToDevice));
      q->h_rtiles = malloc(sizeof(RTile) * rl.size());
      if (!q->h_rtiles) return cosmo_fail(h, COSMO_HIP_ERR_HIP, "out of host memory");
      memcpy(q->h_rtiles, rl.data(), sizeof(RTile) * rl.size());
      HIPCHK(h, hipMalloc((void**)&q->d_rtiles_rep, sizeof(RTile) * rl.size()));
      HIPCHK(h, hipHostMalloc((void**)&q->rep_host, sizeof(RTile) * rl.size()));
      (void)hipFuncSetAttribute((const void*)k_symm_gemm_batch_r<0, 3>, hipFuncAttributeMaxDynamicSharedMemorySize, GemmCfg<64>::SMEM);
      (void)hipFuncSetAttribute((const void*)k_symm_gemm_batch_r<1, 3>, hipFuncAttributeMaxDynamicSharedMemorySize, GemmCfg<64>::SMEM);
      (void)hipFuncSetAttribute((const void*)k_symm_gemm_batch_r<0, 4>, hipFuncAttributeMaxDynamicSharedMemorySize, GemmCfg<64>::SMEM);
      (void)hipFuncSetAttribute((const void*)k_symm_gemm_batch_r<1, 4>, hipFuncAttributeMaxDynamicSharedMemorySize, GemmCfg<64>::SMEM);
    } else {
      for (const BatchCone& bc : q->bcones) { const long long nt = bc.ld / bc.ts; q->batch_flops_performed += 2.0 * (double)(nt * (nt + 1) / 2) * bc.ts * bc.ts * (((bc.d + 31) / 32) * 32); }
    }
    if (tiles.empty()) tiles.push_back(int4{-1, 0, 0, 0});
    HIPCHK(h, hipMalloc((void**)&q->BW, sizeof(real) * (size_t)woff));
    HIPCHK(h, hipMemset(q->BW, 0, sizeof(real) * (size_t)woff));
    HIPCHK(h, hipMalloc((void**)&q->d_bcones, sizeof(BatchCone) * q->bcones.size()));
    HIPCHK(h, hipMalloc((void**)&q->d_btiles, sizeof(int4) * tiles.size()));
    HIPCHK(h, hipMalloc((void**)&q->bparts, sizeof(real) * 3 * BPX * q->bcones.size()));
    HIPCHK(h, hipMalloc((void**)&q->bnrm, sizeof(real) * q->bcones.size()));
    HIPCHK(h, hipMalloc((void**)&q->bgate, sizeof(int) * q->bcones.size()));
    HIPCHK(h, hipMemset(q->bgate, 0, sizeof(int) * q->bcones.size()));
    { const size_t nb = q->bcones.size();
      { int pat = 3; if (const char* e = getenv("COSMO_HIP_POLAR_PATIENCE")) pat = std::max(1, atoi(e));
        q->bk.assign(nb, q->k_lift); q->bstreak.assign(nb, 0); q->bm.assign(nb, pat); }
      HIPCHK(h, hipMalloc((void**)&q->d_lgate, sizeof(int) * nb * POLAR_LIFT_CAP));
      HIPCHK(h, hipMalloc((void**)&q->d_ubuf, sizeof(int) * nb));
      HIPCHK(h, hipHostMalloc((void**)&q->bgate_host, sizeof(int) * nb, hipHostMallocDefault));
      q->lgate_kmax = -1; }
    HIPCHK(h, hipMemcpy(q->d_bcones, q->bcones.data(), sizeof(BatchCone) * q->bcones.size(), hipMemcpyHostToDevice));
    HIPCHK(h, hipMemcpy(q->d_btiles, tiles.data(), sizeof(int4) * tiles.size(), hipMemcpyHostToDevice));
    (void)hipFuncSetAttribute((const void*)k_symm_gemm_batch<0, 3, 64>, hipFuncAttributeMaxDynamicSharedMemorySize, GemmCfg<64>::SMEM);
    (void)hipFuncSetAttribute((const void*)k_symm_gemm_batch<1, 3, 64>, hipFuncAttributeMaxDynamicSharedMemorySize, GemmCfg<64>::SMEM);
    (void)hipFuncSetAttribute((const void*)k_symm_gemm_batch<0, 4, 64>, hipFuncAttributeMaxDynamicSharedMemorySize, GemmCfg<64>::SMEM);
    (void)hipFuncSetAttribute((const void*)k_symm_gemm_batch<1, 4, 64>, hipFuncAttributeMaxDynamicSharedMemorySize, GemmCfg<64>::SMEM);
    (void)hipFuncSetAttribute((const void*)k_symm_gemm_batch<0, 2, 96>, hipFuncAttributeMaxDynamicSharedMemorySize, GemmCfg<96>::SMEM);
    (void)hipFuncSetAttribute((const void*)k_symm_gemm_batch<1, 2, 96>, hipFuncAttributeMaxDynamicSharedMemorySize, GemmCfg<96>::SMEM);
    q->batch_occ = q->batch_ragged ? 4 : 3;
    if (const char* e = getenv("COSMO_HIP_POLAR_BATCH_OCC")) { const int v = atoi(e); if (v == 3 || v == 4) q->batch_occ = v; }
  }
  return COSMO_HIP_OK;
}

bool polar_has_batch(const cosmo_hip_handle* h) { const PolarPlan* q = static_cast<const PolarPlan*>(h->psd_polar); return q && !q->bcones.empty(); }
bool polar_has_large(const cosmo_hip_handle* h) { const PolarPlan* q = static_cast<const PolarPlan*>(h->psd_polar); return q && !q->cones.empty(); }

template <int EPI>
static void launch_bgemm(PolarPlan* q, hipStream_t st, const Ctl* ctl, int guard, const int* gate, int ia, int ib, int icin, int ic, real alpha, real beta) {
  if (q->batch_ragged && q->nrep > 0) {
    if (q->batch_occ == 4)
      hipLaunchKernelGGL((k_symm_gemm_batch_r<EPI, 4>), dim3(q->nrep), dim3(256), GemmCfg<64>::SMEM, st, ctl, guard, gate, (const RTile*)q->d_rtiles_rep, q->d_bcones,
                         q->BW, ia, ib, icin, ic, alpha, beta);
    else
      hipLaunchKernelGGL((k_symm_gemm_batch_r<EPI, 3>), dim3(q->nrep), dim3(256), GemmCfg<64>::SMEM, st, ctl, guard, gate, (const RTile*)q->d_rtiles_rep, q->d_bcones,
                         q->BW, ia, ib, icin, ic, alpha, beta);
    q->repair_launch_tiles += q->nrep;
    return;
  }
  if (q->batch_ragged && q->nrtiles > 0) {
    if (q->batch_occ == 4)
      hipLaunchKernelGGL((k_symm_gemm_batch_r<EPI, 4>), dim3(q->nrtiles), dim3(256), GemmCfg<64>::SMEM, st, ctl, guard, gate, (const RTile*)q->d_rtiles, q->d_bcones,
                         q->BW, ia, ib, icin, ic, alpha, beta);
    else
      hipLaunchKernelGGL((k_symm_gemm_batch_r<EPI, 3>), dim3(q->nrtiles), dim3(256), GemmCfg<64>::SMEM, st, ctl, guard, gate, (const RTile*)q->d_rtiles, q->d_bcones,
                         q->BW, ia, ib, icin, ic, alpha, beta);
    return;
  }
  if (q->nbtiles96 > 0)
    hipLaunchKernelGGL((k_symm_gemm_batch<EPI, 2, 96>), dim3(q->nbtiles96), dim3(256), GemmCfg<96>::SMEM, st, ctl, guard, gate, q->d_btiles + q->nbtiles,
                       q->d_bcones, q->BW, ia, ib, icin, ic, alpha, beta);
  if (q->nbtiles > 0 && q->batch_wave) {
    hipLaunchKernelGGL((k_symm_gemm_batch_w<EPI>), dim3(q->nbtiles), dim3(64), 0, st, ctl, guard, gate, q->d_btiles, q->d_bcones, q->BW, ia, ib, icin, ic, alpha, beta);
  } else if (q->nbtiles > 0) {
    if (q->batch_occ == 4)
      hipLaunchKernelGGL((k_symm_gemm_batch<EPI, 4, 64>), dim3(q->nbtiles), dim3(256), GemmCfg<64>::SMEM, st, ctl, guard, gate, q->d_btiles, q->d_bcones, q->BW,
                         ia, ib, icin, ic, alpha, beta);
    else
      hipLaunchKernelGGL((k_symm_gemm_batch<EPI, 3, 64>), dim3(q->nbtiles), dim3(256), GemmCfg<64>::SMEM, st, ctl, guard, gate, q->d_btiles, q->d_bcones, q->BW,
                         ia, ib, icin, ic, alpha, beta);
  }
}

int32_t polar_enqueue_project_batch(cosmo_hip_handle* h, real* s, int guard) {
  PolarPlan* q = static_cast<PolarPlan*>(h->psd_polar);
  PsdPlan* p = h->psd;
  hipStream_t st = h->stream;
  const int n = (int)q->bcones.size();
  real* vparts = q->bparts + (size_t)2 * BPX * n;
  const bool adapt = q->adapt && !q->speculate && !getenv("COSMO_HIP_POLAR_KLIFT") && q->k_lift <= POLAR_LIFT_CAP;
  int kmax = q->k_lift;
  if (adapt) {
    kmax = 0;
    for (int c = 0; c < n; ++c) kmax = std::max(kmax, q->bk[c]);
    if (q->lgate_kmax != kmax) {
      std::vector<int> lg((size_t)std::max(kmax, 1) * n, 0), ub((size_t)n, 1);
      for (int c = 0; c < n; ++c) {
        const int t0 = kmax - q->bk[c];
        for (int t = t0; t < kmax; ++t) lg[(size_t)t * n + c] = 1;
        ub[(size_t)c] = (t0 & 1) ? 2 : 1;
      }
      HIPCHK(h, hipMemcpyAsync(q->d_lgate, lg.data(), sizeof(int) * lg.size(), hipMemcpyHostToDevice, st));
      HIPCHK(h, hipMemcpyAsync(q->d_ubuf, ub.data(), sizeof(int) * ub.size(), hipMemcpyHostToDevice, st));
      HIPCHK(h, hipStreamSynchronize(st));
      q->lgate_kmax = kmax;
    }
  }
  hipLaunchKernelGGL(k_bpolar_populate, dim3(BPX, n), dim3(COSMO_BS), 0, st, h->ctl, guard, q->d_bcones, s, q->BW, q->bparts);
  hipLaunchKernelGGL(k_bpolar_scale, dim3(BPX, n), dim3(COSMO_BS), 0, st, h->ctl, guard, q->d_bcones, q->bparts, q->BW, q->bnrm, adapt ? (const int*)q->d_ubuf : (const int*)nullptr);
  int iu = 1, iy = 2, products = 0;
  DfArgs dfa;
  bool df = q->dataflow && q->batch_ragged && q->nrtiles > 0 && !adapt && !h->profiling && 3 * (kmax + POLAR_NFIN) + 2 <= DF_MAX_PROD;
  dfa.nprod = 0;
  auto product = [&](int epi, const int* gate, int ia, int ib, int icin, int ic, real alpha, real beta) {
    if (df) { DfProd& pr = dfa.prod[dfa.nprod++]; pr.ia = ia; pr.ib = ib; pr.icin = icin; pr.ic = ic; pr.epi = epi; pr.pad = 0; pr.alpha = alpha; pr.beta = beta; return; }
    if (epi) launch_bgemm<1>(q, st, h->ctl, guard, gate, ia, ib, icin, ic, alpha, beta);
    else launch_bgemm<0>(q, st, h->ctl, guard, gate, ia, ib, icin, ic, alpha, beta);
  };
  auto flush_dataflow = [&]() -> int32_t {
    if (!df) return COSMO_HIP_OK;
    for (int x = 0; x < 9; ++x) dfa.xoff[x] = q->df_xoff[x];
    HIPCHK(h, hipMemsetAsync(q->d_df_sync, 0, sizeof(unsigned) * (DF_SYNC_DONE + q->bcones.size()), st));
    if (!q->df_ev[0]) { HIPCHK(h, hipEventCreate(&q->df_ev[0])); HIPCHK(h, hipEventCreate(&q->df_ev[1])); }
    if (q->df_ev_pending && hipEventQuery(q->df_ev[1]) == hipSuccess) {
      float ms = 0.f;
      if (hipEventElapsedTime(&ms, q->df_ev[0], q->df_ev[1]) == hipSuccess) { q->df_seconds += 1e-3 * (double)ms; q->df_timed += 1; }
      q->df_ev_pending = 0;
    }
    (void)hipGetLastError();
    const bool timed = !q->df_ev_pending;
    if (timed) HIPCHK(h, hipEventRecord(q->df_ev[0], st));
    hipLaunchKernelGGL((k_polar_dataflow<4>), dim3(q->df_grid), dim3(256), GemmCfg<64>::SMEM, st, h->ctl, guard, (const RTile*)q->d_df_tiles, (const int*)q->d_df_cone_nt,
                       q->d_df_sync, q->BW, dfa);
    if (timed) { HIPCHK(h, hipEventRecord(q->df_ev[1], st)); q->df_ev_pending = 1; }
    q->df_launches += 1; q->df_nprod = dfa.nprod;
    df = false;
    return COSMO_HIP_OK;
  };
  auto step = [&](const real* co, const int* gate) {
    product(0, gate, iu, iu, iu, iy, 1.0, 0.0);
    product(1, gate, iy, iy, iy, 3, co[2], co[1]);
    product(1, gate, iu, 3, iu, iy, 1.0, co[0]);
    std::swap(iu, iy);
    products += 3; q->launches[3] += 3;
  };
  auto verify = [&](int round, const int* gate) -> int32_t {
    product(0, gate, iu, 0, 0, 3, 1.0, 0.0);
    product(1, gate, iu, 3, 0, iy, 1.0, -1.0);
    CHK(flush_dataflow());
    hipLaunchKernelGGL(k_bpolar_sumsq, dim3(BPX, n), dim3(COSMO_BS), 0, st, h->ctl, guard, gate, q->d_bcones, q->BW, iy, vparts);
    hipLaunchKernelGGL(k_bpolar_decide, dim3(1), dim3(COSMO_BS), 0, st, h->ctl, guard, q->dev, q->bgate, round, round == q->max_rounds ? 1 : 0, n, q->d_bcones,
                       vparts, q->bnrm, q->tol_factor);
    products += 2; q->launches[3] += 2;
    return COSMO_HIP_OK;
  };
  for (int t = 0; t < kmax; ++t) step(kPolarLift, adapt ? (const int*)(q->d_lgate + (size_t)t * n) : (const int*)nullptr);
  for (int t = 0; t < POLAR_NFIN; ++t) step(kPolarFinish[t], nullptr);
  CHK(verify(0, nullptr));
  q->products_last_batch = products;
  { double wsum = 0.0, w3 = 0.0;
    for (int c = 0; c < n; ++c) { const double d3 = (double)q->bcones[c].d * q->bcones[c].d * q->bcones[c].d; w3 += d3; wsum += d3 * (3.0 * ((adapt ? q->bk[c] : kmax) + POLAR_NFIN) + 2.0); }
    q->wprod_last = w3 > 0.0 ? wsum / w3 : 0.0; }
  for (int r = 1; r <= q->max_rounds; ++r) {
    if (!q->speculate) {
      HIPCHK(h, hipMemcpyAsync(q->gate_host, &q->dev->gate, (adapt && r == 1 ? 5 : 1) * sizeof(int), hipMemcpyDeviceToHost, st));
      if (r == 1 && q->bgate_host) HIPCHK(h, hipMemcpyAsync(q->bgate_host, q->bgate, sizeof(int) * (size_t)n, hipMemcpyDeviceToHost, st));
      HIPCHK(h, hipStreamSynchronize(st));
      if (adapt && r == 1 && q->gate_host[4] != q->seen_proj_batch) {
        q->seen_proj_batch = q->gate_host[4];
        q->depth_proj += 1;
        bool changed = false;
        for (int c = 0; c < n; ++c) {
          if (*q->gate_host && q->bgate_host[c]) {
            q->depth_fail += 1;
            if (q->bk[c] < POLAR_LIFT_CAP) { q->bk[c] += 1; changed = true; }
            q->bstreak[c] = 0;
            q->bm[c] = std::min(96, 2 * q->bm[c]);
          } else if (++q->bstreak[c] >= q->bm[c] && q->bk[c] > 0) {
            q->bk[c] -= 1; q->bstreak[c] = 0; q->depth_down += 1; changed = true;
          }
        }
        if (changed) q->lgate_kmax = -1;
      }
      if (!*q->gate_host) break;
    }
    int rlift = POLAR_RLIFT;
    if (q->compact_repair && q->batch_ragged && q->h_rtiles && q->bgate_host && !q->speculate) {
      if (r == 1) {
        const RTile* all = (const RTile*)q->h_rtiles; RTile* dst = (RTile*)q->rep_host;
        int cnt = 0;
        for (int t = 0; t < q->nrtiles; ++t) if (all[t].cone >= 0 && q->bgate_host[all[t].cone]) dst[cnt++] = all[t];
        if (cnt > 0) {
          HIPCHK(h, hipMemcpyAsync(q->d_rtiles_rep, dst, sizeof(RTile) * (size_t)cnt, hipMemcpyHostToDevice, st));
          q->nrep = cnt; q->repair_trains += 1;
        }
        if (adapt) rlift = 1;
      }
    }
    for (int t = 0; t < rlift; ++t) step(kPolarLift, q->bgate);
    for (int t = 0; t < POLAR_NFIN; ++t) step(kPolarFinish[t], q->bgate);
    CHK(verify(r, q->bgate));
  }
  q->nrep = 0;
  hipLaunchKernelGGL(k_bpolar_finish, dim3(BPX, n), dim3(COSMO_BS), 0, st, h->ctl, guard, q->d_bcones, q->BW, iu, s, q->bparts);
  hipLaunchKernelGGL(k_bpolar_rank, dim3((n + 63) / 64), dim3(64), 0, st, h->ctl, guard, n, q->d_bcones, q->bparts, p->rank);
  HIPCHK(h, hipGetLastError());
  return COSMO_HIP_OK;
}

int32_t polar_enqueue_project(cosmo_hip_handle* h, real* s, int guard) {
  PolarPlan* q = static_cast<PolarPlan*>(h->psd_polar);
  PsdPlan* p = h->psd;
  hipStream_t st = h->stream;
  for (size_t ci = 0; ci < q->cones.size(); ++ci) {
    const PolarCone& cn = q->cones[ci];
    const long long n2 = (long long)cn.ld * cn.ld;
    real* X = q->W + cn.woff;
    real* U = X + n2;
    real* Y = U + n2;
    real* T = Y + n2;
    real* nparts = q->parts + 2 * COSMO_MAX_PARTIALS * ci;
    real* tparts = nparts + COSMO_MAX_PARTIALS;
    const int gpop = std::min(cn.ld, 1024);
    int products = 0;
    hipLaunchKernelGGL(k_polar_populate, dim3(gpop), dim3(COSMO_BS), 0, st, h->ctl, guard, cn, s, X, nparts);
    hipLaunchKernelGGL(k_polar_scale, dim3(1024), dim3(COSMO_BS), 0, st, h->ctl, guard, n2, gpop, nparts, X, U, q->nrm + ci);
    auto step = [&](const real* co, const int* gate) {
      symm_gemm(h, guard, gate, cn.ts, cn.sk, 0, U, U, nullptr, Y, cn.ld, 1.0, 0.0, cn.skg, cn.skc);
      symm_gemm(h, guard, gate, cn.ts, cn.sk, 1, Y, Y, Y, T, cn.ld, co[2], co[1], cn.skg, cn.skc);
      symm_gemm(h, guard, gate, cn.ts, cn.sk, 1, U, T, U, Y, cn.ld, 1.0, co[0], cn.skg, cn.skc);
      std::swap(U, Y);
      products += 3;
    };
    auto verify = [&](int round, const int* gate) {
      symm_gemm(h, guard, gate, cn.ts, cn.sk, 0, U, X, nullptr, T, cn.ld, 1.0, 0.0, cn.skg, cn.skc);
      symm_gemm(h, guard, gate, cn.ts, cn.sk, 1, U, T, X, Y, cn.ld, 1.0, -1.0, cn.skg, cn.skc);
      hipLaunchKernelGGL(k_polar_sumsq, dim3(1024), dim3(COSMO_BS), 0, st, h->ctl, guard, gate, n2, Y, nparts);
      hipLaunchKernelGGL(k_polar_decide, dim3(1), dim3(COSMO_BS), 0, st, h->ctl, guard, q->dev, round, round == q->max_rounds ? 1 : 0, 1024, nparts,
                         q->nrm + ci, q->tol_factor * cn.d * PSD_EPS);
      products += 2;
    };
    const bool adapt = q->adapt && !q->speculate && !getenv("COSMO_HIP_POLAR_KLIFT") && q->k_lift <= POLAR_LIFT_CAP;
    if (adapt && q->lk.size() != q->cones.size()) { q->lk.assign(q->cones.size(), q->k_lift); q->lstreak.assign(q->cones.size(), 0); q->lm.assign(q->cones.size(), 3); }
    int k_main = adapt ? q->lk[ci] : q->k_lift;
    if (q->rescale && k_main > 0) {
      symm_gemm(h, guard, nullptr, cn.ts, cn.sk, 0, U, U, nullptr, Y, cn.ld, 1.0, 0.0, cn.skg, cn.skc);
      hipLaunchKernelGGL(k_polar_sumsq, dim3(1024), dim3(COSMO_BS), 0, st, h->ctl, guard, (const int*)nullptr, n2, Y, nparts);
      hipLaunchKernelGGL(k_polar_rescale, dim3(1024), dim3(COSMO_BS), 0, st, h->ctl, guard, n2, 1024, nparts, U, Y);
      symm_gemm(h, guard, nullptr, cn.ts, cn.sk, 1, Y, Y, Y, T, cn.ld, kPolarLift[2], kPolarLift[1], cn.skg, cn.skc);
      symm_gemm(h, guard, nullptr, cn.ts, cn.sk, 1, U, T, U, Y, cn.ld, 1.0, kPolarLift[0], cn.skg, cn.skc);
      std::swap(U, Y);
      products += 3;
      k_main -= 1;
      if (cn.d >= 1024 && k_main > 1) k_main -= 1;
    }
    for (int t = 0; t < k_main; ++t) step(kPolarLift, nullptr);
    for (int t = 0; t < POLAR_NFIN_LARGE; ++t) step(kPolarFinish[t], nullptr);
    verify(0, nullptr);
    q->products_last_large = products;
    for (int r = 1; r <= q->max_rounds; ++r) {
      if (!q->speculate) {
        HIPCHK(h, hipMemcpyAsync(q->gate_host, &q->dev->gate, (adapt && r == 1 ? 5 : 1) * sizeof(int), hipMemcpyDeviceToHost, st));
        HIPCHK(h, hipStreamSynchronize(st));
        if (adapt && r == 1 && q->gate_host[4] != q->seen_proj_large) {
          q->seen_proj_large = q->gate_host[4];
          q->depth_proj += 1;
          if (*q->gate_host) { q->depth_fail += 1; q->lk[ci] = std::min(POLAR_LIFT_CAP, q->lk[ci] + 1); q->lstreak[ci] = 0; q->lm[ci] = std::min(96, 2 * q->lm[ci]); }
          else if (++q->lstreak[ci] >= q->lm[ci] && q->lk[ci] > 2) { q->lk[ci] -= 1; q->lstreak[ci] = 0; q->depth_down += 1; }
        }
        if (!*q->gate_host) break;
      }
      for (int t = 0; t < POLAR_RLIFT_LARGE; ++t) step(kPolarLift, &q->dev->gate);
      for (int t = 0; t < POLAR_NFIN_LARGE; ++t) step(kPolarFinish[t], &q->dev->gate);
      verify(r, &q->dev->gate);
    }
    const int gfin = std::min(cn.d, 1024);
    hipLaunchKernelGGL(k_polar_finish, dim3(gfin), dim3(COSMO_BS), 0, st, h->ctl, guard, cn, X, T, U, s, tparts);
    hipLaunchKernelGGL(k_polar_rank, dim3(1), dim3(COSMO_BS), 0, st, h->ctl, guard, cn.d, gfin, tparts, p->rank + cn.idx, cn.kind);
  }
  HIPCHK(h, hipGetLastError());
  return COSMO_HIP_OK;
}

int32_t polar_adapt(cosmo_hip_handle* h) {
  PolarPlan* q = static_cast<PolarPlan*>(h->psd_polar);
  if (!q || !q->dev || h->comm || getenv("COSMO_HIP_POLAR_KLIFT")) return COSMO_HIP_OK;
  if (q->adapt && !q->speculate) return COSMO_HIP_OK;
  PolarDev now;
  HIPCHK(h, hipMemcpyAsync(&now, q->dev, sizeof now, hipMemcpyDeviceToHost, h->stream));
// ... 2 lines not shown
  q->seen = now;
  if (dp > 0 && 3 * dr >= dp && q->k_lift < 18) q->k_lift = std::min(18, q->k_lift + 3);
  return COSMO_HIP_OK;
}

extern "C" int32_t cosmo_hip_polar_stats(cosmo_hip_handle* h, int64_t out[16]) {
  if (!h || !out) return COSMO_HIP_ERR_INVALID;
  for (int i = 0; i < 16; ++i) out[i] = 0;
  PolarPlan* q = static_cast<PolarPlan*>(h->psd_polar);
  if (!q) return COSMO_HIP_OK;
  if (hipSetDevice(h->device) != hipSuccess) return cosmo_fail(h, COSMO_HIP_ERR_HIP, "hipSetDevice failed");
  PolarDev now;
  HIPCHK(h, hipMemcpyAsync(&now, q->dev, sizeof now, hipMemcpyDeviceToHost, h->stream));
  HIPCHK(h, hipStreamSynchronize(h->stream));
  out[0] = (int64_t)q->cones.size(); out[1] = (int64_t)q->bcones.size();
  if (!q->cones.empty()) { out[2] = q->cones[0].ts; out[3] = q->cones[0].sk; }
  out[4] = q->launches[0]; out[5] = q->launches[1]; out[6] = q->launches[2]; out[7] = q->launches[3];
  out[8] = q->products_last_large; out[9] = now.rounds; out[10] = now.verified; out[11] = q->products_last_batch;
  out[12] = q->k_lift + POLAR_NFIN; out[13] = now.unverified; out[14] = now.projections;
  out[15] = (int64_t)llround((double)now.err_max * 1e18);
  return COSMO_HIP_OK;
}

extern "C" int32_t cosmo_hip_polar_dataflow_stats(cosmo_hip_handle* h, double out[8]) {
  if (!h || !out) return COSMO_HIP_ERR_INVALID;
  for (int i = 0; i < 8; ++i) out[i] = 0.0;
  PolarPlan* q = static_cast<PolarPlan*>(h->psd_polar);
  if (!q) return COSMO_HIP_OK;
  if (hipSetDevice(h->device) != hipSuccess) return cosmo_fail(h, COSMO_HIP_ERR_HIP, "hipSetDevice failed");
  if (q->df_ev_pending) {
    HIPCHK(h, hipEventSynchronize(q->df_ev[1]));
    float ms = 0.f;
    if (hipEventElapsedTime(&ms, q->df_ev[0], q->df_ev[1]) == hipSuccess) { q->df_seconds += 1e-3 * (double)ms; q->df_timed += 1; }
    q->df_ev_pending = 0;
  }
  out[0] = q->dataflow; out[1] = (double)q->df_launches; out[2] = q->df_nprod; out[3] = (double)q->df_timed;
  out[4] = q->df_timed ? q->df_seconds / (double)q->df_timed : 0.0;
  out[5] = q->batch_flops_performed * q->df_nprod; out[6] = q->df_grid; out[7] = q->df_xoff[8];
  return COSMO_HIP_OK;
}
extern "C" int32_t cosmo_hip_polar_dataflow_reset_timing(cosmo_hip_handle* h) {
  if (!h) return COSMO_HIP_ERR_INVALID;
  PolarPlan* q = static_cast<PolarPlan*>(h->psd_polar);
  if (q) { q->df_seconds = 0.0; q->df_timed = 0; }
  return COSMO_HIP_OK;
}

extern "C" int32_t cosmo_hip_polar_depth_stats(cosmo_hip_handle* h, int64_t out[8]) {
  if (!h || !out) return COSMO_HIP_ERR_INVALID;
  for (int i = 0; i < 8; ++i) out[i] = 0;
  PolarPlan* q = static_cast<PolarPlan*>(h->psd_polar);
  if (!q) return COSMO_HIP_OK;
  const bool adapt = q->adapt && !q->speculate && !getenv("COSMO_HIP_POLAR_KLIFT") && q->k_lift <= POLAR_LIFT_CAP;
  out[0] = adapt ? 1 : 0;
  const std::vector<int>& ks = !q->bk.empty() ? q->bk : q->lk;
  if (adapt && !ks.empty()) {
    long long sum = 0; int mn = ks[0], mx = ks[0];
    for (int v : ks) { sum += v; mn = std::min(mn, v); mx = std::max(mx, v); }
    out[1] = mn; out[2] = mx; out[3] = (1000 * sum) / (long long)ks.size();
  } else { out[1] = out[2] = q->k_lift; out[3] = 1000LL * q->k_lift; }
  out[4] = (int64_t)llround(1000.0 * q->wprod_last);
  out[5] = q->depth_fail; out[6] = q->depth_down; out[7] = q->depth_proj;
  return COSMO_HIP_OK;
}

extern "C" int32_t cosmo_hip_polar_streamk_stats(cosmo_hip_handle* h, int64_t out[4]) {
  if (!h || !out) return COSMO_HIP_ERR_INVALID;
  for (int i = 0; i < 4; ++i) out[i] = 0;
  PolarPlan* q = static_cast<PolarPlan*>(h->psd_polar);
  if (!q || q->cones.empty() || !q->sk_sync) return COSMO_HIP_OK;
  if (hipSetDevice(h->device) != hipSuccess) return cosmo_fail(h, COSMO_HIP_ERR_HIP, "hipSetDevice failed");
  unsigned hdr[2] = {0, 0};
  HIPCHK(h, hipMemcpyAsync(hdr, q->sk_sync, sizeof hdr, hipMemcpyDeviceToHost, h->stream));
  HIPCHK(h, hipStreamSynchronize(h->stream));
  out[0] = 1; out[1] = q->cones[0].skg; out[2] = q->cones[0].skc; out[3] = hdr[1];
  return COSMO_HIP_OK;
}

extern "C" int32_t cosmo_hip_time_psd_product(cosmo_hip_handle* h, int32_t which, int32_t reps, double* avg_seconds, double* flops) {
  if (!h || reps <= 0 || !avg_seconds) return COSMO_HIP_ERR_INVALID;
  PolarPlan* q = static_cast<PolarPlan*>(h->psd_polar);
  if (!q || (which == 0 && q->cones.empty()) || (which != 0 && q->bcones.empty())) return cosmo_fail(h, COSMO_HIP_ERR_INVALID, "time_psd_product: no such cones");
  if (hipSetDevice(h->device) != hipSuccess) return cosmo_fail(h, COSMO_HIP_ERR_HIP, "hipSetDevice failed");
  hipEvent_t e0, e1;
  HIPCHK(h, hipEventCreate(&e0)); HIPCHK(h, hipEventCreate(&e1));
  double fl = 0.0;
  const long long keep[4] = {q->launches[0], q->launches[1], q->launches[2], q->launches[3]};
  for (int pass = 0; pass < 2; ++pass) {
    if (pass == 1) HIPCHK(h, hipEventRecord(e0, h->stream));
    const int R = pass == 0 ? 2 : reps;
    for (int i = 0; i < R; ++i) {
      if (which == 0) {
        const PolarCone& cn = q->cones[0];
        const long long n2 = (long long)cn.ld * cn.ld;
        real* X = q->W + cn.woff;
        symm_gemm(h, 0, nullptr, cn.ts, cn.sk, 0, X + n2, X + n2, nullptr, X + 2 * n2, cn.ld, 1.0, 0.0, cn.skg, cn.skc);
        const long long nt = cn.ld / cn.ts;
        fl = 2.0 * (double)(nt * (nt + 1) / 2) * cn.ts * cn.ts * cn.ld;
      } else if (which == 1) {
        launch_bgemm<0>(q, h->stream, h->ctl, 0, (const int*)nullptr, 1, 1, 1, 2, 1.0, 0.0);
        fl = q->batch_flops_performed;
      } else {
        launch_bgemm<0>(q, h->stream, h->ctl, 0, (const int*)nullptr, 1, 1, 1, 2, 1.0, 0.0);
        launch_bgemm<1>(q, h->stream, h->ctl, 0, (const int*)nullptr, 2, 2, 2, 3, 0.0, 0.0);
        launch_bgemm<1>(q, h->stream, h->ctl, 0, (const int*)nullptr, 1, 3, 1, 2, 1.0, 1.0);
        fl = q->batch_flops_performed;
      }
    }
    if (pass == 1) HIPCHK(h, hipEventRecord(e1, h->stream));
  }
  HIPCHK(h, hipEventSynchronize(e1));
  for (int i = 0; i < 4; ++i) q->launches[i] = keep[i];
  float ms = 0.f;
  HIPCHK(h, hipEventElapsedTime(&ms, e0, e1));
  *avg_seconds = (double)ms * 1e-3 / ((double)reps * (which == 2 ? 3.0 : 1.0));
  if (flops) *flops = fl;
  (void)hipEventDestroy(e0); (void)hipEventDestroy(e1);
  return COSMO_HIP_OK;
}

#define COSMO_CPLX_CHOL_MAX 1024
__global__ __launch_bounds__(COSMO_BS) void k_cplx_chol_pd(int off, int d, const real* __restrict__ vec, real sign, real tol,
                                                           real* __restrict__ G, int* __restrict__ ok_out) {
  __shared__ real rowj[COSMO_CPLX_CHOL_MAX];
  __shared__ real piv;
  __shared__ int fail;
  const real* x = vec + off;
  for (long long e = threadIdx.x; e < (long long)d * d; e += COSMO_BS) {
    const int i = (int)(e % d), j = (int)(e / d);
    real v = sign * polar_read(x, COSMO_HIP_PSD_TRIANGLE_COMPLEX, d, i, j);
    if (i == j) v += tol;
    G[e] = v;
  }
  if (threadIdx.x == 0) fail = 0;
  __syncthreads();
  for (int j = 0; j < d; ++j) {
    for (int k = threadIdx.x; k < j; k += COSMO_BS) rowj[k] = G[(long long)k * d + j];
    __syncthreads();
    for (int i = j + threadIdx.x; i < d; i += COSMO_BS) {
      real v = G[(long long)j * d + i];
      for (int k = 0; k < j; ++k) v -= G[(long long)k * d + i] * rowj[k];
      G[(long long)j * d + i] = v;
      if (i == j) { piv = v; if (!(v > R(0.0))) fail = 1; }
    }
    __syncthreads();
    if (fail) break;
    const real ljj = sqrt(piv);
    for (int i = j + threadIdx.x; i < d; i += COSMO_BS) G[(long long)j * d + i] = (i == j) ? ljj : G[(long long)j * d + i] / ljj;
    __syncthreads();
  }
  if (threadIdx.x == 0) *ok_out = fail ? 0 : 1;
}

int32_t polar_complex_is_pd(cosmo_hip_handle* h, const real* vec, real sign, real tol, std::vector<int>& ok) {
  PsdPlan* p = h->psd;
  ok.clear();
  if (!p || p->cplx.empty()) return COSMO_HIP_OK;
  ok.assign(p->cplx.size(), 0);
  int dmax = 0;
  for (int idx : p->cplx) if (p->cones[idx].d <= COSMO_CPLX_CHOL_MAX) dmax = std::max(dmax, p->cones[idx].d);
  if (dmax == 0) return COSMO_HIP_OK;
  real* G = nullptr; int* d_ok = nullptr;
  HIPCHK(h, hipMalloc((void**)&G, sizeof(real) * (size_t)dmax * dmax));
  if (hipMalloc((void**)&d_ok, sizeof(int)) != hipSuccess) { (void)hipFree(G); return cosmo_fail(h, COSMO_HIP_ERR_HIP, "hipMalloc failed"); }
  int32_t rc = COSMO_HIP_OK;
  for (size_t q = 0; q < p->cplx.size() && rc == COSMO_HIP_OK; ++q) {
// ... 12 lines not shown
```

include/cosmo_hip.h:

```cpp
#ifndef COSMO_HIP_H
#define COSMO_HIP_H

#include <stdint.h>

#ifdef __cplusplus
extern "C" {
#endif

#ifdef COSMO_HIP_REAL_FLOAT
typedef float cosmo_hip_real;
#else
typedef double cosmo_hip_real;
#endif

typedef struct cosmo_hip_handle cosmo_hip_handle;
#if defined(__GNUC__) || defined(__clang__)
#define COSMO_HIP_API __attribute__((visibility("default")))
#else
#define COSMO_HIP_API
#endif

enum {
  COSMO_HIP_OK = 0,
  COSMO_HIP_ERR_INVALID = 1,
// ... 54 lines not shown
  double adaptive_rho_tolerance;
  double cosmo_infty_min_scaling;
  double time_limit;
  int64_t max_iter;
  int64_t adaptive_rho_max_adaptions;
  int32_t kkt_kind;
  int32_t check_termination;
  int32_t check_infeasibility;
  int32_t adaptive_rho;
  int32_t adaptive_rho_interval;
  int32_t unscale_residuals;
  double obj_true;
  double obj_true_tol;
  double adaptive_rho_fraction;
  double setup_time;
} cosmo_hip_params;

enum { COSMO_HIP_ACCEL_EMPTY = 0, COSMO_HIP_ACCEL_ANDERSON = 1,
       COSMO_HIP_ACCEL_ANDERSON_TYPE1_RESTARTED = 2, COSMO_HIP_ACCEL_ANDERSON_TYPE1_ROLLING = 3,
       COSMO_HIP_ACCEL_ANDERSON_TYPE2NE_RESTARTED = 4, COSMO_HIP_ACCEL_ANDERSON_TYPE2NE_ROLLING = 5 };
typedef struct cosmo_hip_accel_params {
  int32_t kind;
  int32_t mem;
  int32_t min_mem;
  int32_t safeguard;
  int64_t start_iter;
  double safeguard_tol;
  double eta_max;
  double start_accuracy;
} cosmo_hip_accel_params;

#define COSMO_HIP_MAX_RHO_UPDATES 64
typedef struct cosmo_hip_result {
  int32_t status;
  int32_t n_rho_updates;
  int64_t iter;
  int64_t kkt_iters_total;
  int64_t kkt_solves;
  double cost;
  double r_prim, r_dual, max_norm_prim, max_norm_dual;
  double rho;
  double iter_time;
  double proj_time;
  double rho_updates[COSMO_HIP_MAX_RHO_UPDATES];
  int64_t safeguarding_iter;
} cosmo_hip_result;

COSMO_HIP_API int32_t cosmo_hip_create(cosmo_hip_handle** h, int32_t device_id);
COSMO_HIP_API int32_t cosmo_hip_destroy(cosmo_hip_handle* h);
COSMO_HIP_API const char* cosmo_hip_last_error(const cosmo_hip_handle* h);
#define COSMO_HIP_ABI_VERSION 1004
COSMO_HIP_API int32_t cosmo_hip_version(void);
COSMO_HIP_API void cosmo_hip_default_params(cosmo_hip_params* p);

COSMO_HIP_API int32_t cosmo_hip_set_problem(cosmo_hip_handle* h, int64_t n, int64_t m,
                              const int64_t* P_colptr, const int64_t* P_rowval, const cosmo_hip_real* P_nzval,
                              const int64_t* A_colptr, const int64_t* A_rowval, const cosmo_hip_real* A_nzval,
                              const cosmo_hip_real* q, const cosmo_hip_real* b);
COSMO_HIP_API int32_t cosmo_hip_set_cones(cosmo_hip_handle* h, int64_t ncones, const int32_t* type, const int64_t* dim,
                            const cosmo_hip_real* box_l, const cosmo_hip_real* box_u);
COSMO_HIP_API int32_t cosmo_hip_set_cones_ex(cosmo_hip_handle* h, int64_t ncones, const int32_t* type, const int64_t* dim,
                               const cosmo_hip_real* box_l, const cosmo_hip_real* box_u, const cosmo_hip_real* cone_param);
typedef void (*cosmo_hip_project_fn)(cosmo_hip_real* x, int64_t dim, void* user);
typedef int32_t (*cosmo_hip_cone_test_fn)(const cosmo_hip_real* x, int64_t dim, double tol, void* user);
COSMO_HIP_API int32_t cosmo_hip_set_custom_cone(cosmo_hip_handle* h, int64_t cone, cosmo_hip_project_fn project, cosmo_hip_cone_test_fn in_dual,
                                  cosmo_hip_cone_test_fn in_pol_recc, void* user);
COSMO_HIP_API int32_t cosmo_hip_set_params(cosmo_hip_handle* h, const cosmo_hip_params* p, const cosmo_hip_real* rho_vec);
COSMO_HIP_API int32_t cosmo_hip_update_rho(cosmo_hip_handle* h, const cosmo_hip_real* rho_vec);
COSMO_HIP_API int32_t cosmo_hip_set_scaling(cosmo_hip_handle* h, const cosmo_hip_real* Dinv, const cosmo_hip_real* Einv, double cinv);
COSMO_HIP_API int32_t cosmo_hip_set_scaling_full(cosmo_hip_handle* h, const cosmo_hip_real* D, const cosmo_hip_real* Dinv, const cosmo_hip_real* E, const cosmo_hip_real* Einv,
                                   double c, double cinv);
COSMO_HIP_API void cosmo_hip_default_accel_params(cosmo_hip_accel_params* p);
COSMO_HIP_API int32_t cosmo_hip_set_accelerator(cosmo_hip_handle* h, const cosmo_hip_accel_params* p);
COSMO_HIP_API int32_t cosmo_hip_get_accel_stats(cosmo_hip_handle* h, int64_t out[6]);
COSMO_HIP_API int32_t cosmo_hip_get_accel_restarts(cosmo_hip_handle* h, int64_t out[2]);
COSMO_HIP_API int32_t cosmo_hip_scale_ruiz(cosmo_hip_handle* h, int64_t iterations, double min_scaling, double max_scaling, cosmo_hip_real* D_out,
                             cosmo_hip_real* E_out, double* c_out);
COSMO_HIP_API int32_t cosmo_hip_update_qb(cosmo_hip_handle* h, const cosmo_hip_real* q, const cosmo_hip_real* b);
COSMO_HIP_API int32_t cosmo_hip_get_rho_classes(cosmo_hip_handle* h, int32_t* cls );
COSMO_HIP_API int32_t cosmo_hip_get_rho_vec(cosmo_hip_handle* h, cosmo_hip_real* rho_vec );

COSMO_HIP_API int32_t cosmo_hip_kkt_solve(cosmo_hip_handle* h, cosmo_hip_real* lhs, const cosmo_hip_real* rhs, int64_t* kkt_iters_out);
COSMO_HIP_API int32_t cosmo_hip_project(cosmo_hip_handle* h, cosmo_hip_real* s, int64_t* psd_rank_out, int32_t* soc_branch_out);
COSMO_HIP_API int32_t cosmo_hip_spmv(cosmo_hip_handle* h, int32_t which, cosmo_hip_real* y, const cosmo_hip_real* x);

COSMO_HIP_API int32_t cosmo_hip_set_iterates(cosmo_hip_handle* h, const cosmo_hip_real* x0, const cosmo_hip_real* s0, const cosmo_hip_real* mu0);
COSMO_HIP_API int32_t cosmo_hip_admm_init(cosmo_hip_handle* h);
COSMO_HIP_API int32_t cosmo_hip_admm_iterate(cosmo_hip_handle* h, int64_t n_iters);
COSMO_HIP_API int32_t cosmo_hip_admm_iterate_checked(cosmo_hip_handle* h, int64_t n_iters, int32_t* status_out);
COSMO_HIP_API int32_t cosmo_hip_residuals(cosmo_hip_handle* h, double out[5]);
COSMO_HIP_API int32_t cosmo_hip_optimize(cosmo_hip_handle* h, cosmo_hip_result* result);
COSMO_HIP_API int32_t cosmo_hip_get_iterates(cosmo_hip_handle* h, cosmo_hip_real* w, cosmo_hip_real* w_prev, cosmo_hip_real* s, cosmo_hip_real* mu);
COSMO_HIP_API int32_t cosmo_hip_cg_persist_stats(cosmo_hip_handle* h, int64_t out[8]);
COSMO_HIP_API int32_t cosmo_hip_get_kkt_solution(cosmo_hip_handle* h, cosmo_hip_real* sol);
COSMO_HIP_API int32_t cosmo_hip_fold_stats(cosmo_hip_handle* h, int64_t out[6]);
COSMO_HIP_API const char* cosmo_hip_kkt_recurrence(cosmo_hip_handle* h);

COSMO_HIP_API int32_t cosmo_hip_ldl_analyze(int64_t n, int64_t m, const int64_t* P_colptr, const int64_t* P_rowval, const int64_t* A_colptr,
                                            const int64_t* A_rowval, const int64_t* perm, int64_t out[8]);
COSMO_HIP_API int32_t cosmo_hip_set_kkt_perm(cosmo_hip_handle* h, int64_t len, const int64_t* perm);
COSMO_HIP_API int32_t cosmo_hip_direct_info(cosmo_hip_handle* h, int64_t out[8]);
COSMO_HIP_API int32_t cosmo_hip_get_stats(cosmo_hip_handle* h, int64_t out[8]);
COSMO_HIP_API int32_t cosmo_hip_set_setup_time(cosmo_hip_handle* h, double seconds);
COSMO_HIP_API int32_t cosmo_hip_get_rho_interval(cosmo_hip_handle* h, int64_t out[2]);

COSMO_HIP_API int32_t cosmo_hip_time_spmv(cosmo_hip_handle* h, int32_t which, int32_t reps, double* avg_seconds,
                            double* algorithmic_bytes);
COSMO_HIP_API int32_t cosmo_hip_set_profiling(cosmo_hip_handle* h, int32_t on);
#define COSMO_HIP_NUM_KERNEL_CLASSES 16
COSMO_HIP_API int32_t cosmo_hip_get_kernel_times(cosmo_hip_handle* h, double seconds[COSMO_HIP_NUM_KERNEL_CLASSES],
                                   int64_t launches[COSMO_HIP_NUM_KERNEL_CLASSES]);
COSMO_HIP_API const char* cosmo_hip_kernel_class_name(int32_t k);
COSMO_HIP_API int32_t cosmo_hip_psd_stats(cosmo_hip_handle* h, int64_t out[4]);
enum { COSMO_HIP_PSD_PROJECTION_SIGN = 0, COSMO_HIP_PSD_PROJECTION_EIGEN = 1 };
COSMO_HIP_API int32_t cosmo_hip_set_psd_projection(cosmo_hip_handle* h, int32_t mode);

COSMO_HIP_API int32_t cosmo_hip_polar_stats(cosmo_hip_handle* h, int64_t out[16]);
COSMO_HIP_API int32_t cosmo_hip_polar_streamk_stats(cosmo_hip_handle* h, int64_t out[4]);
COSMO_HIP_API int32_t cosmo_hip_polar_schedule(int32_t k_lift, double* abc, int32_t* nsteps);
COSMO_HIP_API int32_t cosmo_hip_time_psd_product(cosmo_hip_handle* h, int32_t which, int32_t reps, double* avg_seconds, double* flops);
COSMO_HIP_API int32_t cosmo_hip_polar_dataflow_stats(cosmo_hip_handle* h, double out[8]);
COSMO_HIP_API int32_t cosmo_hip_polar_dataflow_reset_timing(cosmo_hip_handle* h);
COSMO_HIP_API int32_t cosmo_hip_polar_depth_stats(cosmo_hip_handle* h, int64_t out[8]);
COSMO_HIP_API int32_t cosmo_hip_time_krylov(cosmo_hip_handle* h, int32_t reps, double* avg_seconds, double* algorithmic_bytes, int32_t* launches_per_iteration);

COSMO_HIP_API int32_t cosmo_hip_comm_unique_id(uint8_t id[128]);
COSMO_HIP_API int32_t cosmo_hip_comm_init(cosmo_hip_handle* h, int32_t rank, int32_t nranks, const uint8_t id[128]);
COSMO_HIP_API int32_t cosmo_hip_comm_destroy(cosmo_hip_handle* h);
COSMO_HIP_API int32_t cosmo_hip_set_cone_shard(cosmo_hip_handle* h, const int64_t* first_cone);
COSMO_HIP_API int32_t cosmo_hip_comm_selftest(cosmo_hip_handle* h);
COSMO_HIP_API int32_t cosmo_hip_comm_allreduce_check(cosmo_hip_handle* h, int64_t count, int64_t out[6]);
COSMO_HIP_API int32_t cosmo_hip_comm_init_hostshm(cosmo_hip_handle* h, int32_t rank, int32_t nranks, const char* name);
COSMO_HIP_API int32_t cosmo_hip_comm_stats(cosmo_hip_handle* h, int64_t out[4]);
COSMO_HIP_API int32_t cosmo_hip_set_cone_ownership(cosmo_hip_handle* h, int64_t cone_lo, int64_t cone_hi);

COSMO_HIP_API int32_t cosmo_hip_set_row_shard(cosmo_hip_handle* h, const int64_t* first_cone);
COSMO_HIP_API int32_t cosmo_hip_row_shard_info(cosmo_hip_handle* h, int64_t out[6]);
COSMO_HIP_API int32_t cosmo_hip_comm_stats_ex(cosmo_hip_handle* h, int64_t out[8]);

typedef struct cosmo_hip_batch cosmo_hip_batch;
COSMO_HIP_API int32_t cosmo_hip_batch_create(cosmo_hip_batch** b, int32_t device_id, int64_t nprob, int64_t n, int64_t m);
COSMO_HIP_API int32_t cosmo_hip_batch_destroy(cosmo_hip_batch* b);
COSMO_HIP_API const char* cosmo_hip_batch_last_error(const cosmo_hip_batch* b);
COSMO_HIP_API int32_t cosmo_hip_batch_set_problem(cosmo_hip_batch* b, int64_t k, const int64_t* P_colptr, const int64_t* P_rowval,
                                    const cosmo_hip_real* P_nzval, const int64_t* A_colptr, const int64_t* A_rowval,
                                    const cosmo_hip_real* A_nzval, const cosmo_hip_real* q, const cosmo_hip_real* bvec);
COSMO_HIP_API int32_t cosmo_hip_batch_set_cones(cosmo_hip_batch* b, int64_t ncones, const int32_t* type, const int64_t* dim,
                                  const cosmo_hip_real* box_l, const cosmo_hip_real* box_u);
COSMO_HIP_API int32_t cosmo_hip_batch_set_cones_ex(cosmo_hip_batch* b, int64_t ncones, const int32_t* type, const int64_t* dim,
                                     const cosmo_hip_real* box_l, const cosmo_hip_real* box_u, const cosmo_hip_real* cone_param);
COSMO_HIP_API int32_t cosmo_hip_batch_set_scaling(cosmo_hip_batch* b, int64_t k, const cosmo_hip_real* Dinv, const cosmo_hip_real* Einv, double cinv);
COSMO_HIP_API int32_t cosmo_hip_batch_set_accelerator(cosmo_hip_batch* b, const cosmo_hip_accel_params* p);
COSMO_HIP_API int32_t cosmo_hip_batch_get_accel_stats(cosmo_hip_batch* b, int64_t* out);
COSMO_HIP_API int32_t cosmo_hip_batch_set_params(cosmo_hip_batch* b, const cosmo_hip_params* p);
COSMO_HIP_API int32_t cosmo_hip_batch_get_rho_classes(cosmo_hip_batch* b, int64_t k, int32_t* cls );
COSMO_HIP_API int32_t cosmo_hip_batch_set_iterates(cosmo_hip_batch* b, const cosmo_hip_real* x0, const cosmo_hip_real* s0, const cosmo_hip_real* mu0);
COSMO_HIP_API int32_t cosmo_hip_batch_optimize(cosmo_hip_batch* b, cosmo_hip_result* results);
COSMO_HIP_API int32_t cosmo_hip_batch_iterate(cosmo_hip_batch* b, int64_t n_iters, int32_t with_init);
COSMO_HIP_API int32_t cosmo_hip_batch_get_counters(cosmo_hip_batch* b, int64_t* out);
COSMO_HIP_API int32_t cosmo_hip_batch_kernel_info(cosmo_hip_batch* b, int64_t out[8]);
COSMO_HIP_API int32_t cosmo_hip_batch_get_iterates(cosmo_hip_batch* b, int64_t k, cosmo_hip_real* w, cosmo_hip_real* w_prev, cosmo_hip_real* s, cosmo_hip_real* mu);
COSMO_HIP_API int32_t cosmo_hip_batch_set_direct(cosmo_hip_batch* b, int32_t on, const int64_t* perm );
COSMO_HIP_API int32_t cosmo_hip_batch_direct_info(cosmo_hip_batch* b, int64_t out[8]);
COSMO_HIP_API int32_t cosmo_hip_batch_direct_counts(cosmo_hip_batch* b, int64_t* out );
COSMO_HIP_API int32_t cosmo_hip_batch_set_scaling_full(cosmo_hip_batch* b, int64_t k, const cosmo_hip_real* D, const cosmo_hip_real* Dinv, const cosmo_hip_real* E,
                                                       const cosmo_hip_real* Einv, double c, double cinv);
// ... 39 lines not shown
```

Baseline: 358.1.

## Make batched polar PSD projection sync-free and defer rank computation

Removes host round-trips in the batched polar PSD projection. All verification rounds are now enqueued speculatively, gated on the device by per-cone and global gate flags inside the dataflow kernel. The sumsq kernel folds in the decide step through a last-block ticket and resets the sync counters itself, which replaces a memset. Rank trace computation is split out of the finish kernel and deferred until ranks are requested. Populate also gains an XCC-aware cone-to-block mapping. The cost is extra launches of gated rounds that may exit early, plus more complex device-side synchronisation.

```diff
diff --git a/cosmo.jl_amd/_ffi.py b/cosmo.jl_amd/_ffi.py
--- a/cosmo.jl_amd/_ffi.py
+++ b/cosmo.jl_amd/_ffi.py
@@ -81,6 +81,7 @@
     "cosmo_hip_get_rho_vec": (C.c_int32, [C.c_void_p, _PR]),
     "cosmo_hip_kkt_solve": (C.c_int32, [C.c_void_p, _PR, _PR, _PI64]),
     "cosmo_hip_project": (C.c_int32, [C.c_void_p, _PR, _PI64, _PI32]),
+    "cosmo_hip_psd_ranks": (C.c_int32, [C.c_void_p, _PI64]),
     "cosmo_hip_spmv": (C.c_int32, [C.c_void_p, C.c_int32, _PR, _PR]),
     "cosmo_hip_set_iterates": (C.c_int32, [C.c_void_p, _PR, _PR, _PR]),
     "cosmo_hip_admm_init": (C.c_int32, [C.c_void_p]),
@@ -400,6 +401,11 @@
         self._chk(self.lib.cosmo_hip_project(self._h, _dp(s), ranks.ctypes.data_as(_PI64), br.ctypes.data_as(_PI32)))
         return s, ranks[:self.ncones], br[:self.ncones]
 
+    def psd_ranks(self):
+        ranks = np.empty(max(self.ncones, 1), dtype=np.int64)
+        self._chk(self.lib.cosmo_hip_psd_ranks(self._h, ranks.ctypes.data_as(_PI64)))
+        return ranks[:self.ncones]
+
     def spmv(self, which, x):
         nin = {MAT_A: self.n, MAT_AT: self.m, MAT_P: self.n}[which]
         nout = {MAT_A: self.m, MAT_AT: self.n, MAT_P: self.n}[which]
diff --git a/cosmo.jl_amd/csrc/api.hip b/cosmo.jl_amd/csrc/api.hip
--- a/cosmo.jl_amd/csrc/api.hip
+++ b/cosmo.jl_amd/csrc/api.hip
@@ -683,6 +683,15 @@
       if ((h->cones.type[k] == COSMO_HIP_PSD_SQUARE || h->cones.type[k] == COSMO_HIP_PSD_TRIANGLE) && h->cones.dim[k] == 1)
         psd_rank_out[k] = s[h->cones.off[k]] > R(0.0) ? 1 : 0;
   }
+  return COSMO_HIP_OK;
+}
+
+extern "C" int32_t cosmo_hip_psd_ranks(cosmo_hip_handle* h, int64_t* psd_rank_out) {
+  ENTER(h);
+  if (h->row_shard) return cosmo_fail(h, COSMO_HIP_ERR_UNSUPPORTED, "psd_ranks: not available on a row-sharded handle");
+  if (!h->have_cones || !psd_rank_out) return cosmo_fail(h, COSMO_HIP_ERR_INVALID, "psd_ranks: not set up");
+  for (size_t k = 0; k < h->cones.type.size(); ++k) psd_rank_out[k] = -1;
+  CHK(psd_get_ranks(h, psd_rank_out));
   return COSMO_HIP_OK;
 }
 
diff --git a/cosmo.jl_amd/csrc/internal.h b/cosmo.jl_amd/csrc/internal.h
--- a/cosmo.jl_amd/csrc/internal.h
+++ b/cosmo.jl_amd/csrc/internal.h
@@ -363,6 +363,7 @@
 int32_t polar_enqueue_project(cosmo_hip_handle* h, real* s, int guard);
 int32_t polar_enqueue_project_batch(cosmo_hip_handle* h, real* s, int guard);
 int32_t polar_adapt(cosmo_hip_handle* h);
+int32_t polar_flush_ranks(cosmo_hip_handle* h);
 bool polar_has_batch(const cosmo_hip_handle* h);
 bool polar_has_large(const cosmo_hip_handle* h);
 
diff --git a/cosmo.jl_amd/csrc/psd.hip b/cosmo.jl_amd/csrc/psd.hip
--- a/cosmo.jl_amd/csrc/psd.hip
+++ b/cosmo.jl_amd/csrc/psd.hip
@@ -419,6 +419,7 @@
 int32_t psd_get_ranks(cosmo_hip_handle* h, int64_t* rank_per_cone) {
   PsdPlan* p = h->psd;
   if (!p || p->cones.empty()) return COSMO_HIP_OK;
+  CHK(polar_flush_ranks(h));
   std::vector<int> r(p->cones.size());
   int fl[4] = {0, 0, 0, 0};
   HIPCHK(h, hipMemcpyAsync(r.data(), p->rank, r.size() * sizeof(int), hipMemcpyDeviceToHost, h->stream));
diff --git a/cosmo.jl_amd/csrc/psd_polar.hip b/cosmo.jl_amd/csrc/psd_polar.hip
--- a/cosmo.jl_amd/csrc/psd_polar.hip
+++ b/cosmo.jl_amd/csrc/psd_polar.hip
@@ -71,6 +71,8 @@
   int nbtiles = 0, nbtiles96 = 0;
   int speculate = 0;
   int* gate_host = nullptr;
+  int syncfree = 1;
+  int ranks_pending = 0, ranks_iu = 1;
   int batch_wave = 0;
   int batch_ragged = 1;
   void* d_rtiles = nullptr;
@@ -97,6 +99,8 @@
   real* bparts = nullptr;
   real* bnrm = nullptr;
   int* bgate = nullptr;
+  int* d_xcones = nullptr;
+  int xcones_slots = 0;
   int adapt = 0;
   int compact_repair = 1;
   std::vector<int> bk, bstreak, bm;
@@ -777,16 +781,23 @@
 #define DF_MAX_PROD 64
 struct DfArgs { DfProd prod[DF_MAX_PROD]; int nprod; int xoff[9]; };
 #define DF_SYNC_DONE 144
+#define DF_SYNC_TICKET 136
 __device__ __forceinline__ unsigned df_xcc_id() { unsigned x; asm volatile("s_getreg_b32 %0, hwreg(HW_REG_XCC_ID)" : "=s"(x)); return x & 7u; }
 __device__ __forceinline__ unsigned df_ld(const unsigned* p) { return __hip_atomic_load(p, __ATOMIC_RELAXED, __HIP_MEMORY_SCOPE_AGENT); }
 #define DF_RMW(ptr) __hip_atomic_fetch_add((ptr), 1u, __ATOMIC_RELAXED, __HIP_MEMORY_SCOPE_AGENT)
+__global__ __launch_bounds__(64) void k_df_probe(unsigned* __restrict__ seen) {
+  unsigned x; asm volatile("s_getreg_b32 %0, hwreg(HW_REG_XCC_ID)" : "=s"(x));
+  if (threadIdx.x == 0) (void)DF_RMW(seen + (x & 15u));
+}
 template <int OCC>
 __global__ __launch_bounds__(256) __attribute__((amdgpu_waves_per_eu(OCC, OCC))) void k_polar_dataflow(Ctl* __restrict__ ctl, int guard, const RTile* __restrict__ tiles,
-                                                         const int* __restrict__ cone_nt, unsigned* __restrict__ sync, real* __restrict__ W, const DfArgs a) {
+                                                         const int* __restrict__ cone_nt, unsigned* __restrict__ sync, real* __restrict__ W, const DfArgs a,
+                                                         const int* __restrict__ lgate, const int* __restrict__ cgate) {
   extern __shared__ real smem[];
   __shared__ unsigned s_item;
   __shared__ int s_fail;
   if (guard && ctl->halt) return;
+  if (lgate && !*lgate) return;
   const int x = (int)df_xcc_id();
   const int x0 = a.xoff[x];
   const unsigned n_x = (unsigned)(a.xoff[x + 1] - x0);
@@ -809,7 +820,8 @@
     if (item >= total) break;
     const unsigned p = item / n_x, t = item - p * n_x;
     const RTile td = tiles[x0 + t];
-    if (p > 0) {
+    const bool live = !cgate || __builtin_amdgcn_readfirstlane(cgate[td.cone]) != 0;
+    if (live && p > 0) {
       if (wave0) {
         if (threadIdx.x == 0) {
           const unsigned target = p * (unsigned)cone_nt[td.cone];
@@ -828,11 +840,12 @@
     }
     const DfProd pr = a.prod[p];
     auto hook = [&]() { if (wave0) { if (threadIdx.x == 0) nxt = DF_RMW(sync + 16 * x); } };
-    if (pr.epi) ragged_tile<1, OCC, true>(td, W, pr.ia, pr.ib, pr.icin, pr.ic, pr.alpha, pr.beta, smem, hook);
+    if (!live) hook();
+    else if (pr.epi) ragged_tile<1, OCC, true>(td, W, pr.ia, pr.ib, pr.icin, pr.ic, pr.alpha, pr.beta, smem, hook);
     else ragged_tile<0, OCC, true>(td, W, pr.ia, pr.ib, pr.icin, pr.ic, pr.alpha, pr.beta, smem, hook);
     asm volatile("s_waitcnt vmcnt(0)" ::: "memory");
     __syncthreads();
-    prev_cone = td.cone;
+    prev_cone = live ? td.cone : -1;
   }
 }
 #ifdef POLAR_LAB_TIMING
@@ -1052,15 +1065,22 @@
 
 #define BPX 16
 __global__ __launch_bounds__(COSMO_BS) void k_bpolar_populate(const Ctl* __restrict__ ctl, int guard, const BatchCone* __restrict__ cones,
-                                                              const real* __restrict__ s, real* __restrict__ W, real* __restrict__ parts) {
+                                                              const real* __restrict__ s, real* __restrict__ W, real* __restrict__ parts,
+                                                              const int* __restrict__ xcones) {
   if (guard && ctl->halt) return;
   __shared__ real red[COSMO_BS / 64];
-  const BatchCone cn = cones[blockIdx.y];
+  int cone = blockIdx.y, part = blockIdx.x;
+  if (xcones) {
+    const int k = blockIdx.x >> 3;
+    cone = xcones[8 * (k / BPX) + (blockIdx.x & 7)]; part = k % BPX;
+    if (cone < 0) return;
+  }
+  const BatchCone cn = cones[cone];
   const real* x = s + cn.off;
   real* X = W + cn.woff;
   const int d = cn.d, ld = cn.ld;
   real acc = 0.0;
-  for (int j = blockIdx.x; j < ld; j += gridDim.x) {
+  for (int j = part; j < ld; j += BPX) {
     for (int i = threadIdx.x; i < ld; i += COSMO_BS) {
       real v = 0.0;
       if (i < d && j < d) { v = polar_read(x, cn.kind, d, i, j); acc += v * v; }
@@ -1068,7 +1088,7 @@
     }
   }
   acc = block_sum(acc, red);
-  if (threadIdx.x == 0) parts[(size_t)blockIdx.y * 2 * BPX + blockIdx.x] = acc;
+  if (threadIdx.x == 0) parts[(size_t)cone * 2 * BPX + part] = acc;
 }
 __global__ __launch_bounds__(COSMO_BS) void k_bpolar_scale(const Ctl* __restrict__ ctl, int guard, const BatchCone* __restrict__ cones,
                                                            const real* __restrict__ parts, real* __restrict__ W, real* __restrict__ bnrm,
@@ -1086,23 +1106,31 @@
   for (long long i = (long long)blockIdx.x * COSMO_BS + threadIdx.x; i < n2; i += (long long)gridDim.x * COSMO_BS) U[i] = X[i] * inv;
 }
 __global__ __launch_bounds__(COSMO_BS) void k_bpolar_finish(const Ctl* __restrict__ ctl, int guard, const BatchCone* __restrict__ cones,
-                                                            real* __restrict__ W, int iu, real* __restrict__ s, real* __restrict__ parts) {
+                                                            real* __restrict__ W, real* __restrict__ s) {
   if (guard && ctl->halt) return;
+  const BatchCone cn = cones[blockIdx.y];
+  const long long n2 = (long long)cn.ld * cn.ld;
+  const real* X = W + cn.woff;
+  const real* H = W + cn.woff + 3 * n2;
+  real* x = s + cn.off;
+  const int d = cn.d, ld = cn.ld;
+  for (int j = blockIdx.x; j < d; j += gridDim.x) {
+    for (int i = threadIdx.x; i <= j; i += COSMO_BS) {
+      const long long o = (long long)j * ld + i;
+      polar_write(x, cn.kind, d, i, j, (X[o] + H[o]) / R(2.0));
+    }
+  }
+}
+__global__ __launch_bounds__(COSMO_BS) void k_bpolar_trace(const BatchCone* __restrict__ cones, const real* __restrict__ W, int iu, real* __restrict__ parts) {
   __shared__ real red[COSMO_BS / 64];
   const BatchCone cn = cones[blockIdx.y];
   const long long n2 = (long long)cn.ld * cn.ld;
-  const real* X = W + cn.woff;
   const real* U = W + cn.woff + iu * n2;
-  const real* H = W + cn.woff + 3 * n2;
-  real* x = s + cn.off;
   const int d = cn.d, ld = cn.ld;
   real tr = 0.0;
   for (int j = blockIdx.x; j < d; j += gridDim.x) {
     for (int i = threadIdx.x; i <= j; i += COSMO_BS) {
-      const long long o = (long long)j * ld + i;
-      const real v = (X[o] + H[o]) / R(2.0);
-      polar_write(x, cn.kind, d, i, j, v);
-      const real u = U[o];
+      const real u = U[(long long)j * ld + i];
       tr += (i == j) ? (u + u * u) : R(2.0) * u * u;
     }
   }
@@ -1119,30 +1147,18 @@
   rank[cones[c].idx] = (int)llround(tr / (cones[c].kind == COSMO_HIP_PSD_TRIANGLE_COMPLEX ? R(4.0) : R(2.0)));
 }
 
-__global__ __launch_bounds__(COSMO_BS) void k_bpolar_sumsq(const Ctl* __restrict__ ctl, int guard, const int* __restrict__ gate, const BatchCone* __restrict__ cones,
-                                                           const real* __restrict__ W, int ig, real* __restrict__ vparts) {
-  if (guard && ctl->halt) return;
-  if (gate && !gate[blockIdx.y]) return;
-  __shared__ real red[COSMO_BS / 64];
-  const BatchCone cn = cones[blockIdx.y];
-  const long long n2 = (long long)cn.ld * cn.ld;
-  const real* G = W + cn.woff + ig * n2;
-  real acc = 0.0;
-  for (long long i = (long long)blockIdx.x * COSMO_BS + threadIdx.x; i < n2; i += (long long)gridDim.x * COSMO_BS) { const real v = G[i]; acc += v * v; }
-  acc = block_sum(acc, red);
-  if (threadIdx.x == 0) vparts[(size_t)blockIdx.y * BPX + blockIdx.x] = acc;
-}
-__global__ __launch_bounds__(COSMO_BS) void k_bpolar_decide(const Ctl* __restrict__ ctl, int guard, PolarDev* __restrict__ pd, int* __restrict__ bgate, int round,
-                                                            int last, int n, const BatchCone* __restrict__ cones, const real* __restrict__ vparts,
-                                                            const real* __restrict__ bnrm, real tol_factor) {
-  if (guard && ctl->halt) return;
-  if (round > 0 && !pd->gate) return;
-  __shared__ real red[COSMO_BS / 64];
+__device__ __forceinline__ real ld_agent(const real* p) {
+  if constexpr (sizeof(real) == 8) return (real)__longlong_as_double((long long)__hip_atomic_load((const unsigned long long*)p, __ATOMIC_RELAXED, __HIP_MEMORY_SCOPE_AGENT));
+  else return (real)__uint_as_float(__hip_atomic_load((const unsigned*)p, __ATOMIC_RELAXED, __HIP_MEMORY_SCOPE_AGENT));
+}
+template <bool FRESH>
+__device__ __forceinline__ void bpolar_decide_body(PolarDev* __restrict__ pd, int* __restrict__ bgate, int round, int last, int n, const BatchCone* __restrict__ cones,
+                                                   const real* vparts, const real* __restrict__ bnrm, real tol_factor, real* red) {
   real emax = 0.0, nfail = 0.0, nchk = 0.0;
   for (int c = threadIdx.x; c < n; c += COSMO_BS) {
     if (round > 0 && !bgate[c]) continue;
     real g2 = 0.0;
-    for (int k = 0; k < BPX; ++k) g2 += vparts[(size_t)c * BPX + k];
+    for (int k = 0; k < BPX; ++k) g2 += FRESH ? ld_agent(vparts + (size_t)c * BPX + k) : vparts[(size_t)c * BPX + k];
     const real nf = bnrm[c];
     const real err = (nf > R(0.0)) ? R(0.5) * sqrt(g2) / nf : R(0.0);
     const bool ok = !(err > tol_factor * cones[c].d * PSD_EPS);
@@ -1162,6 +1178,48 @@
   else if (last) { pd->unverified += 1; pd->gate = 0; }
   else pd->gate = 1;
   (void)nchk;
+}
+struct DfQueues { int n[8]; };
+__global__ __launch_bounds__(COSMO_BS) void k_bpolar_sumsq(Ctl* __restrict__ ctl, int guard, const int* gate, const BatchCone* __restrict__ cones,
+                                                           const real* __restrict__ W, int ig, real* vparts,
+                                                           PolarDev* pd, int* bgate, int round, int last, int n, const real* __restrict__ bnrm,
+                                                           real tol_factor, unsigned* __restrict__ sync, const DfQueues dq, int nprod) {
+  if (guard && ctl->halt) return;
+  if (pd && round > 0 && !pd->gate) return;
+  __shared__ real red[COSMO_BS / 64];
+  __shared__ int s_last;
+  if (!(gate && !gate[blockIdx.y])) {
+    const BatchCone cn = cones[blockIdx.y];
+    const long long n2 = (long long)cn.ld * cn.ld;
+    const real* G = W + cn.woff + ig * n2;
+    real acc = 0.0;
+    for (long long i = (long long)blockIdx.x * COSMO_BS + threadIdx.x; i < n2; i += (long long)gridDim.x * COSMO_BS) { const real v = G[i]; acc += v * v; }
+    acc = block_sum(acc, red);
+    if (threadIdx.x == 0) vparts[(size_t)blockIdx.y * BPX + blockIdx.x] = acc;
+  }
+  if (!pd) return;
+  if (threadIdx.x == 0) {
+    __threadfence();
+    s_last = (DF_RMW(sync + DF_SYNC_TICKET) == gridDim.x * gridDim.y - 1u) ? 1 : 0;
+  }
+  __syncthreads();
+  if (!s_last) return;
+  __threadfence();
+  bpolar_decide_body<true>(pd, bgate, round, last, n, cones, vparts, bnrm, tol_factor, red);
+  if (threadIdx.x < 8) {
+    const unsigned want = (unsigned)dq.n[threadIdx.x] * (unsigned)nprod;
+    if (df_ld(sync + 16 * threadIdx.x) < want) ctl->error = COSMO_HIP_ERR_HIP;
+  }
+  __syncthreads();
+  for (int i = threadIdx.x; i < DF_SYNC_DONE + n; i += COSMO_BS) sync[i] = 0u;
+}
+__global__ __launch_bounds__(COSMO_BS) void k_bpolar_decide(const Ctl* __restrict__ ctl, int guard, PolarDev* __restrict__ pd, int* __restrict__ bgate, int round,
+                                                            int last, int n, const BatchCone* __restrict__ cones, const real* __restrict__ vparts,
+                                                            const real* __restrict__ bnrm, real tol_factor) {
+  if (guard && ctl->halt) return;
+  if (round > 0 && !pd->gate) return;
+  __shared__ real red[COSMO_BS / 64];
+  bpolar_decide_body<false>(pd, bgate, round, last, n, cones, vparts, bnrm, tol_factor, red);
 }
 
 }
@@ -1191,6 +1249,7 @@
   if (q->d_df_tiles) (void)hipFree(q->d_df_tiles);
   if (q->d_df_cone_nt) (void)hipFree(q->d_df_cone_nt);
   if (q->d_df_sync) (void)hipFree(q->d_df_sync);
+  if (q->d_xcones) (void)hipFree(q->d_xcones);
   if (q->df_ev[0]) { (void)hipEventDestroy(q->df_ev[0]); (void)hipEventDestroy(q->df_ev[1]); }
   if (q->dev) (void)hipFree(q->dev);
   delete q;
@@ -1221,7 +1280,7 @@
   if (const char* e = getenv("COSMO_HIP_POLAR_BATCH_TS96")) q->batch_ts96 = atoi(e) ? 1 : 0;
   if (const char* e = getenv("COSMO_HIP_POLAR_BATCH_WAVE")) q->batch_wave = atoi(e) ? 1 : 0;
   q->speculate = (large_list.size() > 2) ? 1 : 0;
-  if (const char* e = getenv("COSMO_HIP_POLAR_SPECULATE")) q->speculate = atoi(e) ? 1 : 0;
+  if (const char* e = getenv("COSMO_HIP_POLAR_SPECULATE")) { q->speculate = atoi(e) ? 1 : 0; q->syncfree = q->speculate; }
   HIPCHK(h, hipHostMalloc((void**)&q->gate_host, 8 * sizeof(int), hipHostMallocDefault));
   for (int i = 0; i < 8; ++i) q->gate_host[i] = 0;
   if (const char* e = getenv("COSMO_HIP_POLAR_ROUNDS")) q->max_rounds = std::min(8, std::max(0, atoi(e)));
@@ -1323,6 +1382,7 @@
     for (const BatchCone& bc : q->bcones) q->batch_flops_useful += (double)bc.d * bc.d * (bc.d + 1.0);
     if (q->batch_ragged) {
       std::vector<std::vector<RTile>> xl(8);
+      std::vector<std::vector<int>> xc(8);
       long long load[8] = {0, 0, 0, 0, 0, 0, 0, 0};
       for (int ci : order) {
         const BatchCone& bc = q->bcones[ci];
@@ -1331,6 +1391,7 @@
         for (int t = 0; t < nt; ++t) start[t + 1] = start[t] + nb16 / nt + (t < nb16 % nt ? 1 : 0);
         int x = 0;
         for (int t = 1; t < 8; ++t) if (load[t] < load[x]) x = t;
+        xc[x].push_back(ci);
         for (int tj = 0; tj < nt; ++tj)
           for (int ti = 0; ti <= tj; ++ti) {
             const int ei = start[ti + 1] - start[ti], ej = start[tj + 1] - start[tj], dg = (ti == tj) ? 1 : 0;
@@ -1352,6 +1413,17 @@
           return (long long)((t.d + 15) / 16) * (10 * slots + 2) + 125;
         };
         for (int x = 0; x < 8; ++x) std::stable_sort(xl[x].begin(), xl[x].end(), [&](const RTile& a, const RTile& b) { return cost(a) > cost(b); });
+      }
+      int pop_xcd = 1;
+      if (const char* e = getenv("COSMO_HIP_POLAR_POPULATE_XCD")) pop_xcd = atoi(e) ? 1 : 0;
+      if (pop_xcd) {
+        size_t slots = 1;
+        for (int x = 0; x < 8; ++x) slots = std::max(slots, xc[x].size());
+        std::vector<int> lst(8 * slots, -1);
+        for (int x = 0; x < 8; ++x) for (size_t sl = 0; sl < xc[x].size(); ++sl) lst[8 * sl + x] = xc[x][sl];
+        HIPCHK(h, hipMalloc((void**)&q->d_xcones, sizeof(int) * lst.size()));
+        HIPCHK(h, hipMemcpy(q->d_xcones, lst.data(), sizeof(int) * lst.size(), hipMemcpyHostToDevice));
+        q->xcones_slots = (int)slots;
       }
       size_t maxlen = 0;
       for (int x = 0; x < 8; ++x) maxlen = std::max(maxlen, xl[x].size());
@@ -1375,6 +1447,16 @@
         { int nmin = INT32_MAX; for (int x = 0; x < 8; ++x) nmin = std::min(nmin, q->df_xoff[x + 1] - q->df_xoff[x]); q->dataflow = (nmin >= q->df_grid / 8) ? 1 : 0; }
         if (const char* e = getenv("COSMO_HIP_POLAR_DATAFLOW")) q->dataflow = atoi(e) ? 1 : 0;
         if (const char* e = getenv("COSMO_HIP_POLAR_DATAFLOW_GRID")) { const int v = atoi(e); if (v >= 8 && v <= 8192) q->df_grid = v; }
+        HIPCHK(h, hipMemsetAsync(q->d_df_sync, 0, sizeof(unsigned) * (DF_SYNC_DONE + cnt.size()), h->stream));
+        if (q->dataflow) {
+          unsigned seen[16];
+          hipLaunchKernelGGL(k_df_probe, dim3(q->df_grid), dim3(64), 0, h->stream, q->d_df_sync);
+          HIPCHK(h, hipMemcpyAsync(seen, q->d_df_sync, sizeof seen, hipMemcpyDeviceToHost, h->stream));
+          HIPCHK(h, hipStreamSynchronize(h->stream));
+          for (int x = 0; x < 16; ++x) if ((x < 8) != (seen[x] > 0u)) q->dataflow = 0;
+          HIPCHK(h, hipMemsetAsync(q->d_df_sync, 0, sizeof seen, h->stream));
+        }
+        HIPCHK(h, hipStreamSynchronize(h->stream));
         (void)hipFuncSetAttribute((const void*)k_polar_dataflow<4>, hipFuncAttributeMaxDynamicSharedMemorySize, GemmCfg<64>::SMEM); }
       HIPCHK(h, hipMalloc((void**)&q->d_rtiles, sizeof(RTile) * rl.size()));
       HIPCHK(h, hipMemcpy(q->d_rtiles, rl.data(), sizeof(RTile) * rl.size(), hipMemcpyHostToDevice));
@@ -1461,7 +1543,6 @@
 
 int32_t polar_enqueue_project_batch(cosmo_hip_handle* h, real* s, int guard) {
   PolarPlan* q = static_cast<PolarPlan*>(h->psd_polar);
-  PsdPlan* p = h->psd;
   hipStream_t st = h->stream;
   const int n = (int)q->bcones.size();
   real* vparts = q->bparts + (size_t)2 * BPX * n;
@@ -1483,21 +1564,33 @@
       q->lgate_kmax = kmax;
     }
   }
-  hipLaunchKernelGGL(k_bpolar_populate, dim3(BPX, n), dim3(COSMO_BS), 0, st, h->ctl, guard, q->d_bcones, s, q->BW, q->bparts);
+  if (q->d_xcones)
+    hipLaunchKernelGGL(k_bpolar_populate, dim3(8 * BPX * q->xcones_slots), dim3(COSMO_BS), 0, st, h->ctl, guard, q->d_bcones, s, q->BW, q->bparts, (const int*)q->d_xcones);
+  else
+    hipLaunchKernelGGL(k_bpolar_populate, dim3(BPX, n), dim3(COSMO_BS), 0, st, h->ctl, guard, q->d_bcones, s, q->BW, q->bparts, (const int*)nullptr);
   hipLaunchKernelGGL(k_bpolar_scale, dim3(BPX, n), dim3(COSMO_BS), 0, st, h->ctl, guard, q->d_bcones, q->bparts, q->BW, q->bnrm, adapt ? (const int*)q->d_ubuf : (const int*)nullptr);
   int iu = 1, iy = 2, products = 0;
   DfArgs dfa;
   bool df = q->dataflow && q->batch_ragged && q->nrtiles > 0 && !adapt && !h->profiling && 3 * (kmax + POLAR_NFIN) + 2 <= DF_MAX_PROD;
+  const bool syncfree = df && q->syncfree;
+  DfQueues dq;
+  for (int x = 0; x < 8; ++x) dq.n[x] = q->df_xoff[x + 1] - q->df_xoff[x];
   dfa.nprod = 0;
   auto product = [&](int epi, const int* gate, int ia, int ib, int icin, int ic, real alpha, real beta) {
     if (df) { DfProd& pr = dfa.prod[dfa.nprod++]; pr.ia = ia; pr.ib = ib; pr.icin = icin; pr.ic = ic; pr.epi = epi; pr.pad = 0; pr.alpha = alpha; pr.beta = beta; return; }
     if (epi) launch_bgemm<1>(q, st, h->ctl, guard, gate, ia, ib, icin, ic, alpha, beta);
     else launch_bgemm<0>(q, st, h->ctl, guard, gate, ia, ib, icin, ic, alpha, beta);
   };
-  auto flush_dataflow = [&]() -> int32_t {
+  auto flush_dataflow = [&](int round) -> int32_t {
     if (!df) return COSMO_HIP_OK;
     for (int x = 0; x < 9; ++x) dfa.xoff[x] = q->df_xoff[x];
-    HIPCHK(h, hipMemsetAsync(q->d_df_sync, 0, sizeof(unsigned) * (DF_SYNC_DONE + q->bcones.size()), st));
+    if (round > 0) {
+      hipLaunchKernelGGL((k_polar_dataflow<4>), dim3(q->df_grid), dim3(256), GemmCfg<64>::SMEM, st, h->ctl, guard, (const RTile*)q->d_df_tiles, (const int*)q->d_df_cone_nt,
+                         q->d_df_sync, q->BW, dfa, (const int*)&q->dev->gate, (const int*)q->bgate);
+      df = false;
+      return COSMO_HIP_OK;
+    }
+    if (!syncfree) HIPCHK(h, hipMemsetAsync(q->d_df_sync, 0, sizeof(unsigned) * (DF_SYNC_DONE + q->bcones.size()), st));
     if (!q->df_ev[0]) { HIPCHK(h, hipEventCreate(&q->df_ev[0])); HIPCHK(h, hipEventCreate(&q->df_ev[1])); }
     if (q->df_ev_pending && hipEventQuery(q->df_ev[1]) == hipSuccess) {
       float ms = 0.f;
@@ -1508,7 +1601,7 @@
     const bool timed = !q->df_ev_pending;
     if (timed) HIPCHK(h, hipEventRecord(q->df_ev[0], st));
     hipLaunchKernelGGL((k_polar_dataflow<4>), dim3(q->df_grid), dim3(256), GemmCfg<64>::SMEM, st, h->ctl, guard, (const RTile*)q->d_df_tiles, (const int*)q->d_df_cone_nt,
-                       q->d_df_sync, q->BW, dfa);
+                       q->d_df_sync, q->BW, dfa, (const int*)nullptr, (const int*)nullptr);
     if (timed) { HIPCHK(h, hipEventRecord(q->df_ev[1], st)); q->df_ev_pending = 1; }
     q->df_launches += 1; q->df_nprod = dfa.nprod;
     df = false;
@@ -1524,10 +1617,17 @@
   auto verify = [&](int round, const int* gate) -> int32_t {
     product(0, gate, iu, 0, 0, 3, 1.0, 0.0);
     product(1, gate, iu, 3, 0, iy, 1.0, -1.0);
-    CHK(flush_dataflow());
-    hipLaunchKernelGGL(k_bpolar_sumsq, dim3(BPX, n), dim3(COSMO_BS), 0, st, h->ctl, guard, gate, q->d_bcones, q->BW, iy, vparts);
-    hipLaunchKernelGGL(k_bpolar_decide, dim3(1), dim3(COSMO_BS), 0, st, h->ctl, guard, q->dev, q->bgate, round, round == q->max_rounds ? 1 : 0, n, q->d_bcones,
-                       vparts, q->bnrm, q->tol_factor);
+    const int nprod = dfa.nprod;
+    CHK(flush_dataflow(round));
+    const int last = round == q->max_rounds ? 1 : 0;
+    if (syncfree) {
+      hipLaunchKernelGGL(k_bpolar_sumsq, dim3(BPX, n), dim3(COSMO_BS), 0, st, h->ctl, guard, gate, q->d_bcones, q->BW, iy, vparts, q->dev, q->bgate, round, last, n,
+                         q->bnrm, q->tol_factor, q->d_df_sync, dq, nprod);
+    } else {
+      hipLaunchKernelGGL(k_bpolar_sumsq, dim3(BPX, n), dim3(COSMO_BS), 0, st, h->ctl, guard, gate, q->d_bcones, q->BW, iy, vparts, (PolarDev*)nullptr, (int*)nullptr, round,
+                         last, n, q->bnrm, q->tol_factor, (unsigned*)nullptr, dq, 0);
+      hipLaunchKernelGGL(k_bpolar_decide, dim3(1), dim3(COSMO_BS), 0, st, h->ctl, guard, q->dev, q->bgate, round, last, n, q->d_bcones, vparts, q->bnrm, q->tol_factor);
+    }
     products += 2; q->launches[3] += 2;
     return COSMO_HIP_OK;
   };
@@ -1538,7 +1638,17 @@
   { double wsum = 0.0, w3 = 0.0;
     for (int c = 0; c < n; ++c) { const double d3 = (double)q->bcones[c].d * q->bcones[c].d * q->bcones[c].d; w3 += d3; wsum += d3 * (3.0 * ((adapt ? q->bk[c] : kmax) + POLAR_NFIN) + 2.0); }
     q->wprod_last = w3 > 0.0 ? wsum / w3 : 0.0; }
-  for (int r = 1; r <= q->max_rounds; ++r) {
+  if (syncfree) {
+    const long long keep = q->launches[3];
+    for (int r = 1; r <= q->max_rounds; ++r) {
+      df = true; dfa.nprod = 0;
+      for (int t = 0; t < POLAR_RLIFT; ++t) step(kPolarLift, q->bgate);
+      for (int t = 0; t < POLAR_NFIN; ++t) step(kPolarFinish[t], q->bgate);
+      CHK(verify(r, q->bgate));
+    }
+    q->launches[3] = keep;
+  }
+  for (int r = 1; r <= q->max_rounds && !syncfree; ++r) {
     if (!q->speculate) {
       HIPCHK(h, hipMemcpyAsync(q->gate_host, &q->dev->gate, (adapt && r == 1 ? 5 : 1) * sizeof(int), hipMemcpyDeviceToHost, st));
       if (r == 1 && q->bgate_host) HIPCHK(h, hipMemcpyAsync(q->bgate_host, q->bgate, sizeof(int) * (size_t)n, hipMemcpyDeviceToHost, st));
@@ -1579,9 +1689,20 @@
     CHK(verify(r, q->bgate));
   }
   q->nrep = 0;
-  hipLaunchKernelGGL(k_bpolar_finish, dim3(BPX, n), dim3(COSMO_BS), 0, st, h->ctl, guard, q->d_bcones, q->BW, iu, s, q->bparts);
-  hipLaunchKernelGGL(k_bpolar_rank, dim3((n + 63) / 64), dim3(64), 0, st, h->ctl, guard, n, q->d_bcones, q->bparts, p->rank);
+  hipLaunchKernelGGL(k_bpolar_finish, dim3(BPX, n), dim3(COSMO_BS), 0, st, h->ctl, guard, q->d_bcones, q->BW, s);
+  q->ranks_pending = 1; q->ranks_iu = iu;
   HIPCHK(h, hipGetLastError());
+  return COSMO_HIP_OK;
+}
+
+int32_t polar_flush_ranks(cosmo_hip_handle* h) {
+  PolarPlan* q = static_cast<PolarPlan*>(h->psd_polar);
+  if (!q || !q->ranks_pending || q->bcones.empty() || !h->psd) return COSMO_HIP_OK;
+  const int n = (int)q->bcones.size();
+  hipLaunchKernelGGL(k_bpolar_trace, dim3(BPX, n), dim3(COSMO_BS), 0, h->stream, q->d_bcones, q->BW, q->ranks_iu, q->bparts);
+  hipLaunchKernelGGL(k_bpolar_rank, dim3((n + 63) / 64), dim3(64), 0, h->stream, h->ctl, 0, n, q->d_bcones, q->bparts, h->psd->rank);
+  HIPCHK(h, hipGetLastError());
+  q->ranks_pending = 0;
   return COSMO_HIP_OK;
 }
 
@@ -1750,6 +1871,7 @@
   PolarPlan* q = static_cast<PolarPlan*>(h->psd_polar);
   if (!q || (which == 0 && q->cones.empty()) || (which != 0 && q->bcones.empty())) return cosmo_fail(h, COSMO_HIP_ERR_INVALID, "time_psd_product: no such cones");
   if (hipSetDevice(h->device) != hipSuccess) return cosmo_fail(h, COSMO_HIP_ERR_HIP, "hipSetDevice failed");
+  CHK(polar_flush_ranks(h));
   hipEvent_t e0, e1;
   HIPCHK(h, hipEventCreate(&e0)); HIPCHK(h, hipEventCreate(&e1));
   double fl = 0.0;
diff --git a/include/cosmo_hip.h b/include/cosmo_hip.h
--- a/include/cosmo_hip.h
+++ b/include/cosmo_hip.h
@@ -160,6 +160,7 @@
 
 COSMO_HIP_API int32_t cosmo_hip_kkt_solve(cosmo_hip_handle* h, cosmo_hip_real* lhs, const cosmo_hip_real* rhs, int64_t* kkt_iters_out);
 COSMO_HIP_API int32_t cosmo_hip_project(cosmo_hip_handle* h, cosmo_hip_real* s, int64_t* psd_rank_out, int32_t* soc_branch_out);
+COSMO_HIP_API int32_t cosmo_hip_psd_ranks(cosmo_hip_handle* h, int64_t* psd_rank_out);
 COSMO_HIP_API int32_t cosmo_hip_spmv(cosmo_hip_handle* h, int32_t which, cosmo_hip_real* y, const cosmo_hip_real* x);
 
 COSMO_HIP_API int32_t cosmo_hip_set_iterates(cosmo_hip_handle* h, const cosmo_hip_real* x0, const cosmo_hip_real* s0, const cosmo_hip_real* mu0);
```

Measured after the change: 334.3. -6.6%, worse.
